# SIMPLE-BuildingSimulation/heat

Hardware: AMD Instinct MI355X
Metric: surface-node-updates/sec (higher is better)
Workload: dtype f64

## Files before the change

heat_amd/csrc/batch.hip:

```cpp
#include <hip/hip_runtime.h>
#include <rccl/rccl.h>

#include <dlfcn.h>

#include <algorithm>
#include <cmath>
#include <cstdarg>
#include <cstdio>
#include <cstdlib>
#include <cstring>
#include <limits>
#include <mutex>
#include <numeric>
#include <string>
#include <vector>

#include "../../include/heat_amd.h"
#include "kernels.hpp"
#include "layout.hpp"
#include "hostpool.hpp"
#include "plan.hpp"

using namespace heat;

// ... 492 lines not shown
    }

    SideArrays &sa = b->sa;
    sa.sc = b->d_side_const.p;
    sa.dyn = b->d_side_dyn.p;
    sa.out = b->d_side_out.p;
    sa.hs_fix = has_fix ? b->d_hs_fix.p : nullptr;
    sa.zc = b->d_zone_contrib.p;
    sa.S = (int32_t)S;
    sa.wstride = 0;
    sa.site = b->n_sites > 1 ? b->d_site.p : nullptr;
    NodeArrays &na = b->na;
    na.T = b->d_T.p; na.V = b->d_V.p; na.U = b->d_U.p;
    na.cls = b->d_cls.p; na.pal = b->d_pal.p;
    na.pal_stride = p.pal_stride;
    na.pal_ubase = p.pal_ubase;
    na.cavref = b->d_cavref.p; na.cavs = b->d_cavs.p;
    na.alpha_f = b->d_alpha_f.p; na.alpha_b = b->d_alpha_b.p; na.cav = b->d_cav_idx.p; na.mass = b->d_mass.p;
    SlotArrays &sl = b->sl;
    const int64_t *sp = b->d_slots.p;
    sl.hs_f = sp; sl.hs_b = sp + S; sl.flow_f = sp + 2 * S; sl.flow_b = sp + 3 * S;
    sl.solar_f = sp + 4 * S; sl.solar_b = sp + 5 * S; sl.ir_f = sp + 6 * S; sl.ir_b = sp + 7 * S;
    HIP_TRY(hipDeviceSynchronize());
    return HEAT_OK;
}

int select_device(heat_batch *b) {
    HIP_TRY(hipSetDevice(b->device));
    return HEAT_OK;
}

std::vector<FastTile> balanced_rounds(const std::vector<FastTile> &tiles, const std::vector<float> &cost, int n_waves) {
    const size_t n = tiles.size();
    if (n_waves <= 0 || n <= (size_t)n_waves) return tiles;
    std::vector<int32_t> order(n);
    std::iota(order.begin(), order.end(), 0);
    std::stable_sort(order.begin(), order.end(), [&](int32_t a, int32_t b) { return cost[a] > cost[b]; });
    std::vector<std::pair<float, int32_t>> heap(n_waves);
    for (int w = 0; w < n_waves; w++) heap[w] = {0.f, w};
    auto later = [](const std::pair<float, int32_t> &a, const std::pair<float, int32_t> &b) {
        return a.first > b.first || (a.first == b.first && a.second > b.second);
    };
    std::make_heap(heap.begin(), heap.end(), later);
    std::vector<std::vector<int32_t>> mine(n_waves);
    for (int32_t t : order) {
        std::pop_heap(heap.begin(), heap.end(), later);
        auto &top = heap.back();
        mine[top.second].push_back(t);
        top.first += cost[t];
        std::push_heap(heap.begin(), heap.end(), later);
    }
    size_t rounds = 0;
    for (const auto &m : mine) rounds = std::max(rounds, m.size());
    FastTile empty;
    empty.node_base = 0;
    empty.surf_base = 0;
    empty.k = (int16_t)(kStreamKindSmall << kStreamKindShift);
    empty.G = 0;
    std::vector<FastTile> out(rounds * (size_t)n_waves, empty);
    for (int w = 0; w < n_waves; w++)
        for (size_t r = 0; r < mine[w].size(); r++) out[r * (size_t)n_waves + w] = tiles[mine[w][r]];
    return out;
}

int rebuild_unified(heat_batch *b) {
    static const bool off = getenv("HEAT_AMD_NO_UNIFIED") != nullptr;
    auto eligible = [](int c) { return kFastPAL[c] && !(kFastM[c] == 16 && (kFastNM[c] || kFastCAV[c])); };
    static const bool cav_off = getenv("HEAT_AMD_NO_UNIFIED_CAV") != nullptr;
    size_t cap = (size_t)b->n_small_tiles;
    for (int c = 0; c < kNumFast; c++) if (eligible(c)) cap += b->h_tiles_cur[c].size();
    const int waves_light = b->n_cu * 3 * 4, waves_cav = b->n_cu * 2 * 4;
    cap += 2 * (size_t)(waves_light + waves_cav) + 2 * (size_t)(waves_light + waves_cav);
    if (b->d_ucount.n == 0) {
        b->ucount_stride = std::max<size_t>(cap, 1);
        HIP_TRY(b->d_ucount.zeros(2 * b->ucount_stride));
    }
    const int ns = b->n_small_plain_tiles;
    for (int c = 0; c < kNumFast; c++) {
        b->class_has_chunks[c] = false;
        for (const FastTile &ft : b->h_tiles_cur[c]) b->class_has_chunks[c] = b->class_has_chunks[c] || (ft.k & kTileChunkyBit) != 0;
    }
    for (int v = 0; v < 2; v++) {
        std::vector<FastTile> part[kStreamVariants];
        int n_classes = 0, n_cav_classes = 0;
        const int nsc = cav_off ? 0 : (v ? b->n_small_tiles - b->n_small_plain_tiles : b->n_smallcav_stream_tiles);
        for (int j = 0; j < nsc; j++) {
            const GeneralTile &g = b->h_gen_tiles_cur[b->n_small_plain_tiles + j];
            FastTile ft;
            ft.node_base = g.node_base;
            ft.surf_base = g.surf_base;
            ft.k = (int16_t)(kStreamKindSmall << kStreamKindShift);
            ft.G = (int16_t)g.G;
            part[3].push_back(ft);
        }
        for (int mi = 2; mi >= 0; mi--)
            for (int c = mi * 6; c < mi * 6 + 6; c++) {
                if (!eligible(c) || (kFastCAV[c] && cav_off)) continue;
                if (kFastCAV[c]) {
                    const int n = v ? b->n_fast_tiles[c] : b->n_stream_tiles[c];
                    n_cav_classes += n > 0;
                    for (int t = 0; t < n; t++) {
                        FastTile ft = b->h_tiles_cur[c][t];
                        ft.k = (int16_t)((ft.k & (0x1ff | kTileMixedBit | kTileChunkyBit)) | (mi << kStreamKindShift) | (kFastNM[c] ? kStreamNmBit : 0));
                        part[3].push_back(ft);
                    }
                    continue;
                }
                const int n = v ? b->n_fast_tiles[c] : b->n_stream_tiles[c];
                n_classes += n > 0;
                for (int t = 0; t < n; t++) {
                    FastTile ft = b->h_tiles_cur[c][t];
                    const bool chunks = (ft.k & kTileChunkyBit) != 0;
                    ft.k = (int16_t)((ft.k & (0x1ff | kTileMixedBit | kTileChunkyBit)) | (mi << kStreamKindShift) | (kFastNM[c] ? kStreamNmBit : 0));
                    part[mi == 2 ? 0 : (chunks ? 2 : 1)].push_back(ft);
                }
            }
        const bool use = !off && (n_classes + (ns > 0)) >= 2;
        const bool use_cav = !off && !cav_off && (n_cav_classes + (nsc > 0)) >= 2;
        b->n_ulist[v] = 0;
        for (int c = 0; c < kNumFast; c++) b->in_ulist[v][c] = eligible(c) && (kFastCAV[c] ? use_cav : use);
        b->small_in_ulist[v] = use && ns > 0;
        b->smallcav_in_ulist[v] = use_cav && nsc > 0;
        for (int q = 0; q < kStreamVariants; q++) b->ulist_part[v][q][0] = b->ulist_part[v][q][1] = 0;
        if (!use) part[0].clear(), part[1].clear(), part[2].clear();
        if (!use_cav) part[3].clear();
        if (!use && !use_cav) continue;
        static const bool balance_off = getenv("HEAT_AMD_NO_BALANCE") != nullptr;
        auto tile_cost = [&](const FastTile &ft, bool cav) -> float {
            const int kind = (ft.k >> kStreamKindShift) & 3;
            if (kind == kStreamKindSmall) return cav ? 12.f : 3.f;
            const float base = kind == 1 ? 1.f : 0.7f;
            if (cav) return 2.5f * base;
            return (ft.k & kStreamNmBit) ? 2.f * base : base;
        };
        if (use) {
            for (int j = 0; j < ns; j++) {
                const GeneralTile &g = b->h_gen_tiles_cur[j];
                FastTile ft;
                ft.node_base = g.node_base;
                ft.surf_base = g.surf_base;
                ft.k = (int16_t)(kStreamKindSmall << kStreamKindShift);
                ft.G = (int16_t)g.G;
                part[1].push_back(ft);
            }
        }
        for (int q : {1, 3}) {
            if (balance_off || part[q].empty()) continue;
            std::vector<float> cost(part[q].size());
            for (size_t t = 0; t < part[q].size(); t++) cost[t] = tile_cost(part[q][t], q == 3);
            part[q] = balanced_rounds(part[q], cost, q == 1 ? waves_light : waves_cav);
        }
        std::vector<FastTile> all;
        for (int q = 0; q < kStreamVariants; q++) {
            b->ulist_part[v][q][0] = (int)all.size();
            b->ulist_part[v][q][1] = (int)part[q].size();
            all.insert(all.end(), part[q].begin(), part[q].end());
        }
        if (all.size() > b->ucount_stride) return fail(HEAT_E_SIZE, "unified tile list grew beyond its counters");
        b->n_ulist[v] = (int)all.size();
        HIP_TRY(b->d_ulist[v].upload(all));
    }
    return HEAT_OK;
}

void enqueue_surfaces(heat_batch *b, int step_fixed, bool streamed_only = false) {
    int nt[kNumFast];
    for (int c = 0; c < kNumFast; c++) nt[c] = streamed_only ? b->n_stream_tiles[c] : b->n_fast_tiles[c];
    const int ul = streamed_only ? 0 : 1;
    const bool unified = b->n_ulist[ul] > 0;
    static const bool zigzag_off = getenv("HEAT_AMD_NO_ZIGZAG") != nullptr;
    const int rev = (!zigzag_off && (b->sweep_parity++ & 1)) ? 1 : 0;
    int n_small_plain = b->n_small_plain_tiles;
    if (unified) {
        for (int c = 0; c < kNumFast; c++) if (b->in_ulist[ul][c]) nt[c] = 0;
        if (b->small_in_ulist[ul]) n_small_plain = 0;
    }
    int n_launch = 0;
    for (int c = 0; c < kNumFast; c++) n_launch += nt[c] > 0;
    int n_cav_tiles = streamed_only ? b->n_smallcav_stream_tiles : b->n_small_tiles - b->n_small_plain_tiles;
    if (unified && b->smallcav_in_ulist[ul]) n_cav_tiles = 0;
    n_launch += unified;
    n_launch += n_small_plain > 0;
    n_launch += n_cav_tiles > 0;
    n_launch += b->n_gen_tiles > b->n_small_tiles;
    static const bool no_fork = getenv("HEAT_AMD_NO_FORK") != nullptr;
    const bool fork = n_launch > 1 && b->side[0] != nullptr && !no_fork && !b->capturing;
    const int n_side = fork ? std::min(n_launch - 1, (int)heat_batch::kSideStreams) : 0;
    int slot = 0;
    auto next_stream = [&]() -> hipStream_t {
        if (n_side == 0) return b->stream;
        const int s = slot++ % (n_side + 1);
        return s == 0 ? b->stream : b->side[s - 1];
    };
    if (n_side > 0) {
        (void)hipEventRecord(b->ev_fork, b->stream);
        for (int i = 0; i < n_side; i++) (void)hipStreamWaitEvent(b->side[i], b->ev_fork, 0);
    }
    if (unified) {
        hipStream_t us = next_stream();
        static const int order_env = getenv("HEAT_AMD_STREAM_ORDER") ? atoi(getenv("HEAT_AMD_STREAM_ORDER")) : 0;
        const int seq[2][kStreamVariants] = {{3, 1, 2, 0}, {0, 1, 2, 3}};
        for (int qi = 0; qi < kStreamVariants; qi++) {
            const int q = seq[order_env ? 1 : 0][rev ? kStreamVariants - 1 - qi : qi];
            const int first = b->ulist_part[ul][q][0], n = b->ulist_part[ul][q][1];
            if (n > 0)
                launch_surfaces_stream(q, b->d_ulist[ul].p + first, n, b->na, b->gen_base, b->sa, b->d_weather.p, b->d_step.p,
                                       step_fixed, b->d_zone_T.p, b->d_flags.p,
                                       b->d_ucount.p + ul * b->ucount_stride + first, b->n_cu, us, rev);
        }
    }
    double work[kNumFast], total_work = 0.0;
    for (int c = 0; c < kNumFast; c++) {
        work[c] = (double)nt[c] * kFastM[c];
        total_work += work[c];
    }
    total_work += 2.0 * b->n_gen_tiles;
    int order[kNumFast];
    for (int c = 0; c < kNumFast; c++) order[c] = c;
    std::sort(order, order + kNumFast, [&](int x, int y) { return nt[x] > nt[y]; });
    for (int q = 0; q < kNumFast; q++) {
        const int c = order[q];
        if (nt[c] <= 0) continue;
        launch_surfaces_fast(kFastM[c], kFastNM[c] ? (b->class_has_chunks[c] ? 2 : 1) : 0, kFastPAL[c], kFastCAV[c], work[c] / total_work,
                             b->d_fast_tiles[c].p, nt[c], b->na,
                             b->sa, b->d_weather.p, b->d_step.p, step_fixed, b->d_zone_T.p, b->d_flags.p,
                             b->d_nomass_iters.p + b->nm_count_base[c], b->n_cu, next_stream(), rev);
    }
    unsigned long long *cnt = b->d_nomass_iters.p + b->nm_count_base[kNumFast];
    if (n_small_plain > 0)
        launch_surfaces_small(0, b->d_gen_tiles.p, n_small_plain, b->na, b->gen_base, b->sa, b->d_cavs.p,
                              b->d_weather.p, b->d_step.p, step_fixed, b->d_zone_T.p, b->d_flags.p, cnt,
                              next_stream());
    if (n_cav_tiles > 0)
        launch_surfaces_small(1, b->d_gen_tiles.p + b->n_small_plain_tiles, n_cav_tiles,
                              b->na, b->gen_base, b->sa, b->d_cavs.p, b->d_weather.p, b->d_step.p, step_fixed,
                              b->d_zone_T.p, b->d_flags.p, cnt + (size_t)b->n_small_plain_tiles * kWave,
                              next_stream());
    if (b->n_gen_tiles > b->n_small_tiles)
        launch_surfaces_general(b->d_gen_tiles.p + b->n_small_tiles, b->n_gen_tiles - b->n_small_tiles, b->na,
                                b->gen_base, b->sa, b->d_cavs.p, b->d_scratch.p, b->d_weather.p, b->d_step.p,
                                step_fixed, b->d_zone_T.p, b->d_flags.p, cnt + (size_t)b->n_small_tiles * kWave,
                                next_stream());
    for (int i = 0; i < n_side; i++) {
        (void)hipEventRecord(b->ev_join[i], b->side[i]);
        (void)hipStreamWaitEvent(b->stream, b->ev_join[i], 0);
    }
}

void enqueue_zones(heat_batch *b, int mode) {
    const int32_t *zl = b->d_zlist.p;
    int nl = b->n_touched;
    if (mode == 3) { zl = b->d_stream_zones.p; nl = b->n_stream_zones; }
    if (mode == 5) { mode = 3; }
    if (mode == 4) { zl = b->d_zlist_stream.p; nl = b->n_touched_stream; mode = 2; }
    launch_zones(b->d_zone_off.p, b->d_zone_entries.p, b->d_zone_contrib.p, b->d_zone_a0.p, b->d_zone_b0.p,
                 b->d_zone_vol.p, b->d_zone_T.p, b->partial_ptr, (int)b->n_zones, b->dt, b->d_step.p,
                 b->d_flags.p, mode, zl, nl, b->d_slot_of.p, b->n_shared, b->zone_rows, b->stream);
}

int enqueue_fused(heat_batch *b, int n_sub, hipStream_t st, bool streamed_beside = false) {
    FusedArgs fa{};
    {
        static const bool zigzag_off = getenv("HEAT_AMD_NO_ZIGZAG") != nullptr;
        fa.reverse = (!zigzag_off && (b->fused_parity++ & 1)) ? 1 : 0;
    }
    fa.zones = b->d_fzones.p;
    fa.zone_eoff = b->d_fzone_eoff.p;
    fa.slots = b->d_fslots.p;
    fa.side_area = b->d_side_area.p;
    fa.side_lzone = b->d_side_lzone.p;
    fa.a0 = b->d_zone_a0.p;
    fa.b0 = b->d_zone_b0.p;
    fa.vol = b->d_zone_vol.p;
    fa.zone_T = b->d_zone_T.p;
    fa.dt = b->dt;
    fa.n_sub = n_sub;
    fa.gen_tiles = b->d_gen_tiles.p;
    fa.gen_base = b->gen_base;
    fa.small_iters = b->d_nomass_iters.p + b->nm_count_base[kNumFast];
    static const int reserve_env = getenv("HEAT_AMD_FUSED_RESERVE") ? atoi(getenv("HEAT_AMD_FUSED_RESERVE")) : -1;
    const bool beside_exchange = (b->comm != nullptr && b->shared_set && b->n_shared > 0) || reserve_env >= 0 || streamed_beside;
    double streamed_share = 0.0;
    if (streamed_beside) {
        double ns = 4.0 * kWave * (b->n_gen_tiles - (b->n_small_tiles - b->n_small_plain_tiles - b->n_smallcav_stream_tiles)), nf = 0.0;
        for (int c = 0; c < kNumFast; c++) {
            ns += (double)b->n_stream_tiles[c] * kFastM[c] * kWave;
            nf += (double)(b->n_fast_tiles[c] - b->n_stream_tiles[c]) * kFastM[c] * kWave;
        }
        streamed_share = ns / std::max(ns + nf, 1.0);
    }
    const int n_cu = b->n_cu;
    if (beside_exchange && b->d_fqueue.n == 0) HIP_TRY(b->d_fqueue.zeros(kNumFast * 4));
    for (int c = 0; c < kNumFast; c++)
        for (int g2 = 0; g2 < 4; g2++) {
            const int nb = (int)b->h_fblocks[c][g2].size();
            if (nb == 0) continue;
            fa.blocks = b->d_fblocks[c][g2].p;
            fa.n_blocks = nb;
            fa.queue = nullptr;
            int grid = nb;
            if (beside_exchange) {
                const int fw = (g2 & 1) ? 8 : 4;
                static const int room_env = getenv("HEAT_AMD_FUSED_ROOM") ? atoi(getenv("HEAT_AMD_FUSED_ROOM")) : 0;
                const int room = room_env > 0 ? room_env : n_cu * fused_blocks_per_cu(kFastM[c], kFastCAV[c], g2 >> 1, fw, b->na.pal_stride);
                const int reserve = reserve_env >= 0 ? reserve_env
                                                     : std::min(room / 2, std::max(fw == 4 ? 16 : 8, (int)(room * streamed_share)));
                if (nb > room - reserve) {
                    grid = std::max(1, room - reserve);
                    fa.queue = b->d_fqueue.p + c * 4 + g2;
                    HIP_TRY(hipMemsetAsync(fa.queue, 0, sizeof(unsigned int), st));
                }
            }
            static const bool trace = getenv("HEAT_AMD_TRACE") != nullptr;
            if (trace)
                fprintf(stderr, "heat_amd: fused launch%s: %d workgroups for %d blocks (class %d, list %d, %d sub-timesteps)\n",
                        fa.queue ? " on the work queue" : "", grid, nb, c, g2, n_sub);
            b->n_fused_launches++;
            const int nm_variant = kFastNM[c] ? ((b->class_has_chunks[c] && !(g2 >> 1) && !kFastCAV[c] && kFastM[c] <= 8) ? 2 : 1) : 0;
            HIP_TRY(launch_surfaces_fused(kFastM[c], nm_variant, kFastCAV[c], g2 >> 1, (g2 & 1) ? 8 : 4, grid, b->d_fast_tiles[c].p, b->n_fast_tiles[c],
                                          b->na, b->sa, b->d_weather.p, b->d_flags.p,
                                          b->d_nomass_iters.p + b->nm_count_base[c], fa, st));
        }
    for (int c = 0; c < kNumFast; c++) {
        const int n_super = (int)b->h_team_supers[c].size();
        if (n_super == 0) continue;
        if (n_sub > 4095) return fail(HEAT_E_INVALID_ARG, "a march call of %d sub-timesteps: the team exchange tags 4095 at most", n_sub);
        static const int team_room_env = getenv("HEAT_AMD_TEAM_ROOM") ? atoi(getenv("HEAT_AMD_TEAM_ROOM")) : 0;
        const int room = team_room_env > 0 ? team_room_env : n_cu * std::min(2, fused_team_blocks_per_cu(kFastM[c], kFastNM[c], b->na.pal_stride));
        int team_size = 2;
        for (const FusedSuper &su : b->h_team_supers[c]) team_size = std::max(team_size, (int)su.n_members);
        const int n_teams = std::min(n_super, std::max(0, room - room / 8) / team_size);
        if (n_teams >= 1 && (n_super + n_teams - 1) / n_teams > 1023)
            return fail(HEAT_E_SIZE, "%d clusters for %d teams: the exchange tags 1023 rounds per launch at most", n_super, n_teams);
        if (n_teams < 1) return fail(HEAT_E_DEVICE, "the device holds %d workgroups of the team variant: not one team", room);
        if (b->xbuf_teams < n_teams) {
            HIP_TRY(b->d_xbuf.zeros((size_t)n_teams * 2 * kTeamZones * kTeamMax * 4));
            b->xbuf_teams = n_teams;
        }
        b->team_epoch++;
        if ((b->team_epoch & 1023u) == 0) {
            HIP_TRY(hipMemsetAsync(b->d_xbuf.p, 0, b->d_xbuf.n * sizeof(unsigned long long), st));
            b->team_epoch++;
        }
        fa.blocks = b->d_team_blocks[c].p;
        fa.n_blocks = (int)b->h_team_blocks[c].size();
        fa.queue = nullptr;
        fa.supers = b->d_team_supers[c].p;
        fa.n_super = n_super;
        fa.team_zinfo = b->d_team_zinfo.p;
        fa.xbuf = b->d_xbuf.p;
        fa.tag_base = (b->team_epoch & 1023u) << 22;
        fa.team_size = team_size;
        static const bool trace = getenv("HEAT_AMD_TRACE") != nullptr;
        if (trace)
            fprintf(stderr, "heat_amd: team launch: %d teams of %d workgroups for %d clusters (class %d, %d sub-timesteps)\n",
                    n_teams, team_size, n_super, c, n_sub);
        b->n_fused_launches++;
        HIP_TRY(launch_surfaces_fused(kFastM[c], kFastNM[c], 0, 2, 4, n_teams * team_size, b->d_fast_tiles[c].p, b->n_fast_tiles[c], b->na,
                                      b->sa, b->d_weather.p, b->d_flags.p, b->d_nomass_iters.p + b->nm_count_base[c], fa, st));
    }
    return HEAT_OK;
}

hipEvent_t next_event(heat_batch *b) {
    if (b->ev_used == b->ev_pool.size()) {
        hipEvent_t e;
        if (hipEventCreate(&e) != hipSuccess) return nullptr;
        b->ev_pool.push_back(e);
    }
    return b->ev_pool[b->ev_used++];
}

struct MarchGuard {
    heat_batch *b;
    double *saved_partial;
    bool forked = false, joined = false;
    explicit MarchGuard(heat_batch *b_) : b(b_), saved_partial(b_->partial_ptr) {}
    ~MarchGuard() {
        b->partial_ptr = saved_partial;
        if (forked && !joined && b->fused_stream) (void)hipStreamSynchronize(b->fused_stream);
    }
};

struct SeriesDrain {
    heat_batch *b;
    ~SeriesDrain() { (void)hipStreamSynchronize(b->stream); }
};

template <typename T>
int series_upload(DevBuf<T> &buf, const T *src, size_t count, const char *what) {
    hipError_t e = buf.alloc(count);
    if (e == hipSuccess && count > 0) e = hipMemcpy(buf.p, src, count * sizeof(T), hipMemcpyHostToDevice);
    if (e != hipSuccess)
        return fail(HEAT_E_DEVICE, "series march: %s (%zu bytes) on the device: %s — nothing has been marched", what, count * sizeof(T),
                    hipGetErrorString(e));
    return HEAT_OK;
}

struct ReportDev {
    DevBuf<uint8_t> gbuf, prev;
    DevBuf<uint32_t> gidx, seg, part_off;
    DevBuf<double> gw, part, group_trace, applied_row;
    DevBuf<double> f64[7];
    DevBuf<int64_t> i64[4];
    DevBuf<double> th_f64[2];
    DevBuf<int64_t> th_i64[3];
};

struct IdealDev {
    DevBuf<int32_t> i32;
    DevBuf<double> cap;
    DevBuf<double> step;
    DevBuf<double> q;
    DevBuf<double> f64[4];
    DevBuf<int64_t> i64[4];
};

struct SkyDev {
    DevBuf<uint8_t> mode;
    DevBuf<double> normal;
    DevBuf<SkyRecord> record;
};
static_assert(sizeof(SkyRecord) == sizeof(heat_sky_record) && sizeof(heat_sky_record) == 64, "SkyRecord mirrors heat_sky_record");

struct GainsDev {
    DevBuf<int32_t> ap_dev;
    DevBuf<double> ap_f64;
    DevBuf<double2> power;
    DevBuf<double> sum;
    DevBuf<double> transmitted;
    DevBuf<uint32_t> rec;
    DevBuf<int64_t> slice_off;
    DevBuf<int32_t> ap;
    DevBuf<double> share;
};

struct AirDev {
    DevBuf<int32_t> i32;
    DevBuf<double> f64;
    DevBuf<uint8_t> state;
    DevBuf<double> sum_q;
    DevBuf<int64_t> i64[2];
    DevBuf<double> path_q;
};

struct ShadeDev {
    DevBuf<double> tab;
    DevBuf<int32_t> i32;
    DevBuf<double> tan2;
    DevBuf<double> f;
    DevBuf<int32_t> side;
    DevBuf<int32_t> aperture;
    DevBuf<double> sunlit;
};

struct RadiationDev {
    DevBuf<uint32_t> face;
    DevBuf<double> emission;
    DevBuf<uint32_t> rec;
    DevBuf<int32_t> off, src;
    DevBuf<double> factor;
    DevBuf<double> sum;
    DevBuf<double> irradiance;
};

template <typename T>
int series_alloc(DevBuf<T> &buf, size_t count, const char *what) {
    const hipError_t e = buf.alloc(count);
    if (e != hipSuccess)
        return fail(HEAT_E_DEVICE, "series march: %s (%zu bytes) on the device: %s — nothing has been marched", what, count * sizeof(T),
                    hipGetErrorString(e));
    return HEAT_OK;
}
template <typename T>
int report_array(DevBuf<T> &buf, const T *host, size_t count, bool upload, const char *what) {
    if (!host) return HEAT_OK;
    return upload ? series_upload(buf, host, count, what) : series_alloc(buf, count, what);
}

}

extern "C" {


int heat_batch_create(const heat_batch_desc *desc, heat_batch **out) {
    heat_batch_options opt;
    memset(&opt, 0, sizeof opt);
    opt.device = -1;
    opt.n_ranks = 1;
    return heat_batch_create_ex(desc, &opt, out);
}

static int create_impl(const heat_batch_desc *desc, const heat_batch_options *opt_in, int32_t n_sites,
                       const int32_t *site_of_surface, bool sites, heat_batch **out) {
    if (!out) return fail(HEAT_E_INVALID_ARG, "out is NULL");
    *out = nullptr;
    heat_batch_options opt;
    memset(&opt, 0, sizeof opt);
    opt.device = -1;
    opt.n_ranks = 1;
    if (opt_in) opt = *opt_in;
    if (sites) {
        std::string err;
        const int rc = check_sites(desc, opt, n_sites, site_of_surface, err);
        if (rc) return fail(rc, "%s", err.c_str());
    }
    if (opt.n_ranks < 1) opt.n_ranks = 1;
    if (opt.nodes_per_lane != 0 && opt.nodes_per_lane != 4 && opt.nodes_per_lane != 8 && opt.nodes_per_lane != 16)
        return fail(HEAT_E_INVALID_ARG, "nodes_per_lane must be 0, 4, 8 or 16");
    int rc;
    {
        std::string err;
        rc = check_desc(desc, err);
        if (rc) return fail(rc, "%s", err.c_str());
    }

    int ndev = 0;
    if (hipGetDeviceCount(&ndev) != hipSuccess || ndev == 0)
        return fail(HEAT_E_DEVICE, "no HIP device available: this library has no CPU fallback");
    heat_batch *b = new heat_batch();
    if (opt.device >= 0) {
        b->device = opt.device;
    } else if (hipGetDevice(&b->device) != hipSuccess) {
        delete b;
        return fail(HEAT_E_DEVICE, "hipGetDevice failed");
    }
    b->n_ranks = opt.n_ranks;
    b->rank = opt.rank;
    b->use_graph = opt.use_graph != 0;
    b->fusion_on = opt.no_fusion != 1;
    rc = select_device(b);
    if (!rc) {
        hipDeviceProp_t prop;
        if (hipGetDeviceProperties(&prop, b->device) == hipSuccess && prop.multiProcessorCount > 0) b->n_cu = prop.multiProcessorCount;
    }
    if (!rc) {
        if (opt.stream) {
            b->stream = reinterpret_cast<hipStream_t>(opt.stream);
        } else {
            hipError_t e = hipStreamCreateWithFlags(&b->stream, hipStreamNonBlocking);
            if (e != hipSuccess) rc = fail(HEAT_E_DEVICE, "hipStreamCreate failed: %s", hipGetErrorString(e));
            b->own_stream = true;
        }
    }
    if (!rc) {
        for (int i = 0; i < heat_batch::kSideStreams && !rc; i++) {
            if (hipStreamCreateWithFlags(&b->side[i], hipStreamNonBlocking) != hipSuccess ||
                hipEventCreateWithFlags(&b->ev_join[i], hipEventDisableTiming) != hipSuccess)
                rc = fail(HEAT_E_DEVICE, "side stream creation failed");
        }
        if (!rc && hipStreamCreateWithFlags(&b->fused_stream, hipStreamNonBlocking) != hipSuccess)
            rc = fail(HEAT_E_DEVICE, "side stream creation failed");
        if (!rc && (hipEventCreateWithFlags(&b->ev_fork, hipEventDisableTiming) != hipSuccess ||
                    hipEventCreateWithFlags(&b->ev_fused, hipEventDisableTiming) != hipSuccess))
            rc = fail(HEAT_E_DEVICE, "event creation failed");
    }
    if (!rc) rc = build(b, desc, opt, n_sites, site_of_surface);
    if (rc) {
        delete b;
        return rc;
    }
    *out = b;
    return HEAT_OK;
}

int heat_batch_create_ex(const heat_batch_desc *desc, const heat_batch_options *opt, heat_batch **out) {
    return create_impl(desc, opt, 1, nullptr, false, out);
}

int heat_batch_create_sites(const heat_batch_desc *desc, const heat_batch_options *opt, int32_t n_sites,
                            const int32_t *site_of_surface, heat_batch **out) {
    return create_impl(desc, opt, n_sites, site_of_surface, true, out);
}

int32_t heat_batch_n_sites(const heat_batch *b) { return b ? b->n_sites : 0; }

int heat_batch_create_shard(const heat_batch_desc *desc, const heat_batch_options *opt, const int32_t *rank_of_surface,
                            heat_batch **out) {
    if (!desc || !opt || !rank_of_surface || !out) return fail(HEAT_E_INVALID_ARG, "NULL argument");
    {
        std::string err;
        const int rc = check_desc(desc, err);
        if (rc) return fail(rc, "%s", err.c_str());
    }
    for (int64_t s = 0; s < desc->n_surfaces; s++)
        if (rank_of_surface[s] < 0 || rank_of_surface[s] >= std::max(opt->n_ranks, 1))
            return fail(HEAT_E_SIZE, "surface %lld: rank %d outside [0, %d)", (long long)s, rank_of_surface[s], std::max(opt->n_ranks, 1));
    ShardDesc sh;
    sh.build(desc, rank_of_surface, opt->rank);
    int rc = heat_batch_create_ex(&sh.desc, opt, out);
    if (rc) return rc;
    heat_batch *b = *out;
    const int64_t Z = desc->n_zones;
    const int n_ranks = std::max(opt->n_ranks, 1);
    std::vector<int32_t> first(Z, -1);
    std::vector<uint8_t> shared(Z, 0), owned(Z, 0);
    auto touch = [&](int32_t z, int32_t rk) {
        if (first[z] < 0) first[z] = rk;
        else if (first[z] != rk) shared[z] = 1;
    };
    for (int64_t s = 0; s < desc->n_surfaces; s++) {
        if (desc->front_kind[s] == HEAT_BOUNDARY_SPACE) touch(desc->front_zone[s], rank_of_surface[s]);
        if (desc->back_kind[s] == HEAT_BOUNDARY_SPACE) touch(desc->back_zone[s], rank_of_surface[s]);
    }
    int64_t n_shared = 0;
    for (int64_t z = 0; z < Z; z++) {
        n_shared += shared[z];
// ... 1508 lines not shown
```

heat_amd/csrc/device_math.hpp:

```cpp
#pragma once
#include <hip/hip_runtime.h>
#include "layout.hpp"

namespace heat {

constexpr double kPi = 3.14159265358979323846264338327950288;

__device__ __forceinline__ double tarp_natural(double air_t, double surf_t, double cos_tilt, int &bad) {
    const double delta_t = air_t - surf_t;
    const double adt = fabs(delta_t);
    const double act = fabs(cos_tilt);
    const double c3 = cbrt(adt);
    double h;
    if (adt < 1e-3 || act < 1e-3) {
        h = 1.31 * c3;
    } else if ((delta_t < 0. && cos_tilt < 0.) || (delta_t > 0. && cos_tilt > 0.)) {
        h = 9.482 * c3 / (7.238 - act);
    } else if ((delta_t > 0. && cos_tilt < 0.) || (delta_t < 0. && cos_tilt > 0.)) {
        h = 1.81 * c3 / (1.382 + act);
    } else {
        bad |= FLAG_UNREACHABLE;
        h = __builtin_nan("");
    }
    return (h < 0.1) ? 0.1 : h;
}

__device__ __forceinline__ double tarp_natural_coef(double air_t, double surf_t, double nat_pos, double nat_neg, int &bad) {
    const double delta_t = air_t - surf_t;
    const double adt = fabs(delta_t);
    const double c3 = cbrt(adt);
    double coef = (delta_t > 0.) ? nat_pos : nat_neg;
    if (adt < 1e-3) coef = 1.31;
    if (delta_t != delta_t || nat_pos != nat_pos) {
        bad |= FLAG_UNREACHABLE;
        coef = __builtin_nan("");
    }
    const double h = coef * c3;
    return (h < 0.1) ? 0.1 : h;
}

__device__ __forceinline__ double tarp_forced(double air_speed, double area, double perimeter, bool windward) {
    const double wf = windward ? 1.0 : 0.5;
    return 2.537 * wf * 1.67 * sqrt(perimeter * air_speed / area);
}

__device__ __forceinline__ bool is_windward(double sin_wd, double cos_wd, double cos_tilt, double nx, double ny) {
    return (fabs(cos_tilt) < 0.98) ? ((nx * sin_wd + ny * cos_wd) > 0.0) : true;
}

__device__ __forceinline__ double ir_to_rad_temperature(double ir) {
    return sqrt(sqrt(ir / kSigma)) - 273.15;
}

__device__ __forceinline__ double clamp_solar_front(double s) { return (s != s || s < 0.0) ? 0.0 : s; }
__device__ __forceinline__ double clamp_solar_back(double s) { return (s != s) ? 0.0 : s; }

__device__ __forceinline__ double rad_hs(double emis, double rad_t, double surf_t) {
    const double tm = 273.15 + (rad_t + surf_t) / 2.;
    return 4. * emis * kSigma * ((tm * tm) * tm);
}

__device__ __forceinline__ void gas_coeffs(int gas, double &k0, double &k1, double &m0, double &m1,
                                           double &c0, double &c1, double &mass) {
    switch (gas) {
    case 1: k0 = 2.285e-3; k1 = 5.149e-5; m0 = 3.379e-6; m1 = 6.451e-8; c0 = 521.9285; c1 = 0.; mass = 39.948; break;
    case 2: k0 = 9.443e-4; k1 = 2.826e-5; m0 = 2.213e-6; m1 = 7.777e-8; c0 = 248.0907; c1 = 0.; mass = 83.8; break;
    case 3: k0 = 4.538e-4; k1 = 1.723e-5; m0 = 1.069e-6; m1 = 7.414e-8; c0 = 158.3397; c1 = 0.; mass = 131.30; break;
    default: k0 = 2.873e-3; k1 = 7.760e-5; m0 = 3.723e-6; m1 = 4.94e-8; c0 = 1002.7370; c1 = 1.2324e-2; mass = 28.97; break;
    }
}

__device__ __forceinline__ double air_density(double temp_k) {
    return 101325. * 28.97 / (8314.46261815324 * temp_k);
}
__device__ __forceinline__ double air_heat_capacity(double temp_k) {
    return 1002.7370 + 1.2324e-2 * temp_k;
}
__device__ __forceinline__ double zone_mcp(double volume, double temp) {
    return volume * air_density(temp + 273.15) * air_heat_capacity(temp + 273.15) / 1.;
}

__device__ __forceinline__ double powr(double x, double y) { return exp(y * log(x)); }

__device__ __attribute__((noinline)) double nu_90(double ra, double a_gi, int &bad) {
    double nu1;
    if (ra <= 1e4) {
        nu1 = 1. + 1.7596678 * 1e-10 * powr(ra, 2.2984755);
    } else if (ra < 5e4) {
        nu1 = 0.028154 * powr(ra, 0.4134);
    } else if (ra > 5e4) {
        nu1 = 0.0673838 * cbrt(ra);
    } else {
        bad |= FLAG_UNREACHABLE;
        nu1 = __builtin_nan("");
    }
    const double nu2 = 0.242 * powr(ra / a_gi, 0.272);
    return (nu1 > nu2) ? nu1 : nu2;
}

__device__ __attribute__((noinline)) double nu_60(double ra, double a_gi) {
    const double g = 0.5 / powr(1. + powr(ra / 3160., 20.6), 0.1);
    const double t = 0.0936 * powr(ra, 0.314) / (1. + g);
    const double t2 = t * t, t4 = t2 * t2;
    const double t7 = (t * t2) * t4;
    const double nu1 = powr(1. + t7, 1. / 7.);
    const double nu2 = (0.104 + 0.175 / a_gi) * powr(ra, 0.283);
    return (nu1 > nu2) ? nu1 : nu2;
}

__device__ __attribute__((noinline)) double nusselt(double ra, double gamma, double a_gi, int &bad) {
    const double THIRTY_RAD = 30. * kPi / 180.;
    const double EPSILON_RAD = 0.5 * kPi / 180.;
    gamma = fmod(gamma, kPi);
    if (gamma >= 0.0 && gamma < 2. * THIRTY_RAD - EPSILON_RAD) {
        const double cos_gamma = cos(gamma);
        const double x = 1. - 1708. / (ra * cos_gamma);
        const double a = (x + fabs(x)) / 2.;
        const double b = 1. - 1708. * powr(sin(1.8 * gamma), 1.6) / (ra * cos_gamma);
        const double c = cbrt(ra * cos_gamma / 5830.) - 1.;
        return 1. + 1.44 * a * b + (c + fabs(c)) / 2.;
    } else if (gamma < 2. * THIRTY_RAD + EPSILON_RAD) {
        return nu_60(ra, a_gi);
    } else if (gamma < 3. * THIRTY_RAD - EPSILON_RAD) {
        const double nu60 = nu_60(ra, a_gi);
        const double nu90 = nu_90(ra, a_gi, bad);
        const double x = (gamma - kPi / 3.) / (kPi / 2. - kPi / 3.);
        return nu60 + (nu90 - nu60) * x;
    } else if (gamma < 3. * THIRTY_RAD + EPSILON_RAD) {
        return nu_90(ra, a_gi, bad);
    } else if (gamma < 6. * THIRTY_RAD) {
        const double nu_v = nu_90(ra, a_gi, bad);
        return 1. + (nu_v - 1.) * sin(gamma);
    }
    bad |= FLAG_UNREACHABLE;
    return __builtin_nan("");
}

__device__ inline double cavity_u_value(const CavityDev &c, double t_front, double t_back, int &bad) {
    double k0, k1, m0, m1, c0, c1, mass;
    gas_coeffs(c.gas, k0, k1, m0, m1, c0, c1, mass);
    double gamma = c.angle;
    if (t_front > t_back) gamma = 180. * (kPi / 180.) - gamma;
    const double a_gi = c.height / c.thickness;
    const double temp = ((t_front + 273.15) + (t_back + 273.15)) / 2.;
    const double lambda = k0 + k1 * temp;
    double ra;
    if (fabs(t_front - t_back) < 1e-10) {
        ra = 0.0000001;
    } else {
        const double beta = 1. / temp;
        const double c_p = (c1 != 0.) ? c0 + c1 * temp : c0;
        const double mu = m0 + m1 * temp;
        const double rho = 101325. * mass / (8314.46261815324 * temp);
        const double th = c.thickness;
        ra = (rho * rho) * ((th * th) * th) * 9.81 * beta * c_p * fabs(t_front - t_back) / (mu * lambda);
    }
    const double nu = nusselt(ra, gamma, a_gi, bad);
    const double conv = nu * lambda / c.thickness;
    const double tm = (t_back + t_front) / 2. + 273.15;
    const double rad = 4. * ((tm * tm) * tm) * kSigma * c.ein * c.eout / (1. - (1. - c.ein) * (1. - c.eout));
    return rad + conv;
}

}
```

heat_amd/csrc/kernels.hip:

```cpp
#include <hip/hip_runtime.h>

#include <algorithm>
#include <atomic>
#include <cstdlib>

#include "device_math.hpp"
#include "kernels.hpp"
#include "layout.hpp"

namespace heat {

__device__ __forceinline__ void eval_side(const SideConst &c, const StepWeather &w, double air_t, double rad_alt,
                                          double rad_out, double surf_t, double &hs, double &rad_t, int &bad) {
    const double natural = tarp_natural(air_t, surf_t, c.cos_eff, bad);
    if ((c.kind_n & 3) == KIND_OUTDOOR) {
        const bool windward = (c.kind_n & 4) ? true : ((c.nx * w.sin_wd + c.ny * w.cos_wd) > 0.0);
        const double wf = windward ? 1.0 : 0.5;
        hs = wf * (c.forced * w.sqrt_ws) + natural;
        rad_t = rad_out;
    } else {
        hs = natural;
        rad_t = rad_alt;
    }
}

typedef __attribute__((address_space(4))) const int32_t ConstInt32;
__device__ __forceinline__ int tile_site(const SideArrays &sd, int surf_base) {
    const ConstInt32 *site = (const ConstInt32 *)sd.site;
    return __builtin_amdgcn_readfirstlane(site[__builtin_amdgcn_readfirstlane(surf_base)]);
}
__device__ __forceinline__ const StepWeather *site_weather(const StepWeather *weather, const SideArrays &sd, int surf_base) {
    if (sd.site == nullptr) return weather;
    return weather + (int64_t)tile_site(sd, surf_base) * sd.wstride;
}

__device__ __forceinline__ double boundary_temperature(const SideConst &c, const StepWeather &w,
                                                       const double *__restrict__ zone_T) {
    const int kind = c.kind_n & 3;
    if (kind == KIND_SPACE) return zone_T[c.zone];
    if (kind == KIND_AMBIENT) return c.ambient;
    return w.t_out;
}

__device__ __forceinline__ long long side_entry_pos(const SideConst &c) { return __double_as_longlong(c.ambient); }
__device__ __forceinline__ void put_zone_contrib(const SideArrays &sd, const SideConst &c, double hs, double t_face) {
    if ((c.kind_n & 3) == KIND_SPACE) {
        ZoneContrib z;
        z.ha = hs * c.forced;
        z.t_face = t_face;
        sd.zc[side_entry_pos(c)] = z;
    }
}

__device__ __forceinline__ void report_failure(int *flags, int bad, unsigned int index) {
    atomicOr(flags, bad);
    atomicMin(reinterpret_cast<unsigned long long *>(flags + 2), ((unsigned long long)index << 8) | (unsigned int)(bad & 0xff));
}

__device__ __forceinline__ double shfl_f64(double v, int src_lane) { return __shfl(v, src_lane, kWave); }

template <int CTRL>
__device__ __forceinline__ double dpp_rotate_f64(double v) {
    int lo = __double2loint(v), hi = __double2hiint(v);
    lo = __builtin_amdgcn_update_dpp(0, lo, CTRL, 0xf, 0xf, false);
    hi = __builtin_amdgcn_update_dpp(0, hi, CTRL, 0xf, 0xf, false);
    return __hiloint2double(hi, lo);
}
template <int CTRL, int ROW_MASK>
__device__ __forceinline__ double dpp_add_f64(double v) {
    int lo = __double2loint(v), hi = __double2hiint(v);
    lo = __builtin_amdgcn_update_dpp(0, lo, CTRL, ROW_MASK, 0xf, true);
    hi = __builtin_amdgcn_update_dpp(0, hi, CTRL, ROW_MASK, 0xf, true);
    return v + __hiloint2double(hi, lo);
}
__device__ __forceinline__ double wave_sum_f64(double v) {
    v = dpp_add_f64<0x111, 0xf>(v);
    v = dpp_add_f64<0x112, 0xf>(v);
    v = dpp_add_f64<0x114, 0xf>(v);
    v = dpp_add_f64<0x118, 0xf>(v);
    v = dpp_add_f64<0x142, 0xa>(v);
    v = dpp_add_f64<0x143, 0xc>(v);
    const int lo = __builtin_amdgcn_readlane(__double2loint(v), 63);
    const int hi = __builtin_amdgcn_readlane(__double2hiint(v), 63);
    return __hiloint2double(hi, lo);
}

__device__ __forceinline__ double row_sum_f64(double v) {
    v = dpp_add_f64<0x111, 0xf>(v);
    v = dpp_add_f64<0x112, 0xf>(v);
    v = dpp_add_f64<0x114, 0xf>(v);
    v = dpp_add_f64<0x118, 0xf>(v);
    return v;
}

__device__ __forceinline__ double from_prev_lane(double v) { return dpp_rotate_f64<0x13C>(v); }
__device__ __forceinline__ double from_next_lane(double v) { return dpp_rotate_f64<0x134>(v); }

template <int M, bool AFFINE, typename VF, typename QF, typename PUT>
__device__ __forceinline__ void apply_A(const double (&x)[M], VF V, const double (&Ue)[M], double ULe, bool is_first,
                                        bool is_last, double qF, QF qsel, PUT put) {
    const double xl_raw = from_prev_lane(x[M - 1]);
    const double xr_raw = from_next_lane(x[0]);
    const double xl = is_first ? 0.0 : xl_raw;
    const double xr = is_last ? 0.0 : xr_raw;
    double fprev = ULe * (x[0] - xl);
    if (AFFINE) fprev -= qF;
#pragma unroll
    for (int j = 0; j < M; j++) {
        const double xj = x[j];
        double f = Ue[j] * (((j == M - 1) ? xr : x[j + 1]) - xj);
        if (AFFINE) f += qsel(j);
        put(j, V(j) * (f - fprev));
        fprev = f;
    }
}

template <int M, typename VF, typename QF>
__device__ __forceinline__ void rk4_horner(double (&T)[M], VF V, const double (&Ue)[M], double ULe, bool is_first,
                                           bool is_last, double qF, QF qsel) {
    double v[M], z[M];
    apply_A<M, true>(T, V, Ue, ULe, is_first, is_last, qF, qsel, [&](int j, double y) { v[j] = y * (1.0 / 24.0); });
    apply_A<M, false>(v, V, Ue, ULe, is_first, is_last, qF, qsel, [&](int j, double y) { z[j] = 4.0 * v[j] + y; });
    apply_A<M, false>(z, V, Ue, ULe, is_first, is_last, qF, qsel, [&](int j, double y) { z[j] = 12.0 * v[j] + y; });
    apply_A<M, false>(z, V, Ue, ULe, is_first, is_last, qF, qsel,
                      [&](int j, double y) { T[j] = (T[j] + 24.0 * v[j]) + y; });
}

#pragma clang fp contract(off)
constexpr int kSmallNodes = 4;
__device__ __forceinline__ double opaque_select(bool cond, double x, double y) {
    const unsigned long long m = __builtin_amdgcn_ballot_w64(cond);
    int lo, hi;
    asm("v_cndmask_b32 %0, %1, %2, %3" : "=v"(lo) : "v"(__double2loint(y)), "v"(__double2loint(x)), "s"(m));
    asm("v_cndmask_b32 %0, %1, %2, %3" : "=v"(hi) : "v"(__double2hiint(y)), "v"(__double2hiint(x)), "s"(m));
    return __hiloint2double(hi, lo);
}
struct Nodes4 {
    double a, b, c, d;
    __device__ __forceinline__ double get(int j) const { return j == 0 ? +a : (j == 1 ? +b : (j == 2 ? +c : +d)); }
    __device__ __forceinline__ void set(int j, double v) {
        if (j == 0) a = v;
        else if (j == 1) b = v;
        else if (j == 2) c = v;
        else d = v;
    }
    __device__ __forceinline__ double last(int nn) const {
        double r = a;
        r = opaque_select(nn == 2, b, r);
        r = opaque_select(nn == 3, c, r);
        r = opaque_select(nn == 4, d, r);
        return r;
    }
};

template <int CAV>
__device__ __forceinline__ void small_step(const SideConst &cf, const SideConst &cb, const SideDyn &df, const SideDyn &db,
                                           const double *__restrict__ hs_fix, int d, int S, const StepWeather &w,
                                           double t_front_b, double t_back_b, int nn, Nodes4 &T,
                                           const double (&Us)[kSmallNodes], const double (&sol)[kSmallNodes],
                                           const int (&cav)[kSmallNodes], const CavityDev (&cv)[kSmallNodes - 1], int &bad,
                                           unsigned int &iters, SideOut &of, SideOut &ob) {
    constexpr int NS = kSmallNodes;
    const int bk = cb.kind_n & 3;
    auto last = [&](const double (&x)[NS]) {
        double r = x[0];
#pragma unroll
        for (int j = 1; j < NS; j++) r = (j == nn - 1) ? +x[j] : +r;
        return r;
    };
    const double T0 = T.a, Tn = T.last(nn);
    const bool quirk = (bk == KIND_AMBIENT);
    double f_hs, f_rad, b_hs, b_rad;
    const double f_surf = T0, b_surf = quirk ? T0 : Tn;
    eval_side(cf, w, t_front_b, t_front_b, df.rad_t, f_surf, f_hs, f_rad, bad);
    eval_side(cb, w, t_back_b, quirk ? t_front_b : t_back_b, db.rad_t, b_surf, b_hs, b_rad, bad);
    if (f_hs != f_hs || b_hs != b_hs) bad |= FLAG_NAN_HS;
    if (hs_fix != nullptr) {
        const double ff = hs_fix[d], fb = hs_fix[S + d];
        if (ff == ff) f_hs = ff;
        if (fb == fb) b_hs = fb;
    }
    const double f_radhs = rad_hs(cf.emis, f_rad, f_surf);
    const double b_radhs = rad_hs(cb.emis, b_rad, b_surf);

    double old_err = 99999.;
    int count = 0;
    for (;;) {
        double lo[NS], dg[NS], up[NS], q[NS];
#pragma unroll
        for (int j = 0; j < NS; j++) { lo[j] = 0.0; dg[j] = 0.0; up[j] = 0.0; q[j] = 0.0; }
#pragma unroll
        for (int j = 0; j < NS - 1; j++) {
            if (j < nn - 1) {
                double u = Us[j];
                if constexpr (CAV) {
                    if (cav[j] >= 0) u = cavity_u_value(cv[j], T.get(j), T.get(j + 1), bad);
                }
                dg[j] += -u;
                dg[j + 1] = dg[j + 1] - u;
                up[j] = up[j] + u;
                lo[j + 1] = lo[j + 1] + u;
            }
        }
        q[0] += t_front_b * f_hs + f_radhs * (f_rad - T.a);
        dg[0] += -f_hs;
        const double bq = t_back_b * b_hs + b_radhs * (b_rad - T.last(nn));
#pragma unroll
        for (int j = 0; j < NS; j++) {
            if (j == nn - 1) { q[j] += bq; dg[j] += -b_hs; }
        }
        iters++;
#pragma unroll
        for (int j = 0; j < NS; j++) q[j] = (q[j] + sol[j]) * -1.;
#pragma unroll
        for (int j = 1; j < NS; j++) {
            if (j < nn) {
                const double f = lo[j] / dg[j - 1];
                dg[j] -= f * up[j - 1];
                q[j] -= f * q[j - 1];
            }
        }
        double x[NS];
#pragma unroll
        for (int j = NS - 1; j >= 0; j--) {
            if (j == nn - 1) x[j] = q[j] / dg[j];
            else if (j < nn - 1) x[j] = (q[j] - up[j] * x[(j + 1) % NS]) / dg[j];
            else x[j] = 0.0;
        }
        double err = 0.0;
#pragma unroll
        for (int j = 0; j < NS; j++) if (j < nn) err += fabs(x[j] - T.get(j));
        if (err > old_err) break;
        if (err != err) { bad |= FLAG_NAN_NOMASS; break; }
#pragma unroll
        for (int j = 0; j < NS; j++) if (j < nn) T.set(j, (T.get(j) + x[j]) * 0.5);
        const double tol = (count < 100) ? 0.01 : 0.5;
        if (err / (double)nn < tol) break;
        old_err = err;
        count++;
    }

    {
        const double T0n = T.a, Tnn = T.last(nn);
        double fh, bh, r_;
        eval_side(cf, w, t_front_b, t_front_b, df.rad_t, T0n, fh, r_, bad);
        eval_side(cb, w, t_back_b, t_back_b, db.rad_t, quirk ? T0n : Tnn, bh, r_, bad);
        if (fh != fh || bh != bh) bad |= FLAG_NAN_HS;
        if (hs_fix != nullptr) {
            const double ff = hs_fix[d], fb = hs_fix[S + d];
            if (ff == ff) fh = ff;
            if (fb == fb) bh = fb;
        }
        of.hs = fh; of.flow = (T0n - t_front_b) * fh;
        ob.hs = bh; ob.flow = (Tnn - t_back_b) * bh;
    }
}

template <int CAV>
__device__ __forceinline__ void small_load(const GeneralTile &tile, int lane, const NodeArrays &na, int64_t gen_base,
                                           const SideDyn &df, const SideDyn &db, int nn, Nodes4 &T,
                                           double (&Us)[kSmallNodes], double (&sol)[kSmallNodes], int (&cav)[kSmallNodes],
                                           CavityDev (&cv)[kSmallNodes - 1]) {
    const double *Tg = na.T + tile.node_base + lane;
    const double *Ug = na.U + tile.node_base + lane;
    const int64_t gofs = tile.node_base - gen_base + lane;
    double tl[kSmallNodes], ul[kSmallNodes], af[kSmallNodes], ab[kSmallNodes];
    int cl[kSmallNodes];
#pragma unroll
    for (int j = 0; j < kSmallNodes; j++) {
        const int64_t jc = (int64_t)min(j, nn - 1) * kWave;
        tl[j] = Tg[jc];
        ul[j] = Ug[jc];
        af[j] = na.alpha_f[gofs + jc];
        ab[j] = na.alpha_b[gofs + jc];
        cl[j] = CAV ? na.cav[gofs + jc] : -1;
    }
#pragma unroll
    for (int j = 0; j < kSmallNodes; j++) {
        const bool v = j < nn;
        T.set(j, v ? tl[j] : 0.0);
        Us[j] = v ? ul[j] : 0.0;
        cav[j] = (CAV && v) ? cl[j] : -1;
        double sj = v ? af[j] * df.solar : 0.0;
        sj += v ? ab[j] * db.solar : 0.0;
        sol[j] = sj;
    }
#pragma unroll
    for (int j = 0; j < kSmallNodes - 1; j++) {
        cv[j] = CavityDev{0., 0., 0., 0., 0., 0, 0};
        if constexpr (CAV) {
            if (cav[j] >= 0) cv[j] = na.cavs[cav[j]];
        }
    }
}

template <int CAV>
__device__ __forceinline__ unsigned int small_tile_march(int64_t node_base, int surf_base, int G, int lane,
                                                         const NodeArrays &na, int64_t gen_base, const SideArrays &sd,
                                                         const StepWeather &w, const double *__restrict__ zone_T,
                                                         int *__restrict__ flags) {
    if (lane >= G) return 0;
    GeneralTile tile;
    tile.node_base = node_base;
    tile.surf_base = surf_base;
    tile.G = G;
    const int d = surf_base + lane;
    const int S = sd.S;
    const SideConst cf = sd.sc[d];
    const SideConst cb = sd.sc[S + d];
    const SideDyn df = sd.dyn[d];
    const SideDyn db = sd.dyn[S + d];
    const int nn = cf.kind_n >> 16;
    Nodes4 T{0.0, 0.0, 0.0, 0.0};
    double Us[kSmallNodes], sol[kSmallNodes];
    int cav[kSmallNodes];
    CavityDev cv[kSmallNodes - 1];
    small_load<CAV>(tile, lane, na, gen_base, df, db, nn, T, Us, sol, cav, cv);
    int bad = 0;
    unsigned int iters = 0;
    SideOut of, ob;
    small_step<CAV>(cf, cb, df, db, sd.hs_fix, d, S, w, boundary_temperature(cf, w, zone_T),
                    boundary_temperature(cb, w, zone_T), nn, T, Us, sol, cav, cv, bad, iters, of, ob);
    double *Tg = na.T + node_base + lane;
#pragma unroll
    for (int j = 0; j < kSmallNodes; j++) if (j < nn) Tg[(int64_t)j * kWave] = T.get(j);
    sd.out[d] = of;
    sd.out[S + d] = ob;
    {
        const double Tl = T.last(nn);
        put_zone_contrib(sd, cf, of.hs, T.a);
        put_zone_contrib(sd, cb, ob.hs, Tl);
    }
    if (bad) report_failure(flags, bad, (unsigned int)d);
    return iters;
}

template <int CAV>
__global__ void __launch_bounds__(256, 2)
k_surfaces_small(const GeneralTile *__restrict__ tiles, int n_tiles, NodeArrays na, int64_t gen_base,
                 SideArrays sd, const CavityDev *__restrict__ cavs,
                 const StepWeather *__restrict__ weather, const int *__restrict__ step_ptr, int step_fixed,
                 const double *__restrict__ zone_T, int *__restrict__ flags,
                 unsigned long long *__restrict__ nomass_iters) {
    const int lane = threadIdx.x & (kWave - 1);
    const int wave = blockIdx.x * (blockDim.x >> 6) + (threadIdx.x >> 6);
    if (wave >= n_tiles) return;
    const GeneralTile tile = tiles[wave];
    const int step = (step_fixed >= 0) ? step_fixed : *step_ptr;
    const StepWeather w = site_weather(weather, sd, tile.surf_base)[step];
    const unsigned int iters = small_tile_march<CAV>(tile.node_base, tile.surf_base, tile.G, lane, na, gen_base, sd, w, zone_T, flags);
    if (lane < tile.G) nomass_iters[(int64_t)wave * kWave + lane] += iters;
}
#pragma clang fp contract(fast)

struct FusedLds {
    double2 *hT;
    double *zT, *za0, *zb0, *zvol;
    double *zsa, *zsb;
    int *zoff;
    unsigned short *slots;
};

constexpr int kFusedBarriersAtInit = 1;
constexpr int kFusedBarriersPerSubstep = 2;

__device__ __forceinline__ void fused_block_init(const FusedBlock &blk, const FusedArgs &fa, const FusedLds &l, int n_threads) {
    const int e_first = fa.zone_eoff[blk.first_zone];
    if ((int)threadIdx.x <= blk.n_zones) l.zoff[threadIdx.x] = fa.zone_eoff[blk.first_zone + threadIdx.x] - e_first;
    if ((int)threadIdx.x < blk.n_zones) {
        const int z = fa.zones[blk.first_zone + threadIdx.x];
        l.zT[threadIdx.x] = fa.zone_T[z];
        l.za0[threadIdx.x] = fa.a0[z];
        l.zb0[threadIdx.x] = fa.b0[z];
        l.zvol[threadIdx.x] = fa.vol[z];
    }
    const int n_e = fa.zone_eoff[blk.first_zone + blk.n_zones] - e_first;
    for (int e = threadIdx.x; e < n_e; e += n_threads) l.slots[fa.slots[e_first + e]] = (unsigned short)e;
    __syncthreads();
}

struct FusedPre {
    int e_first, n_e, zoff, z, slot0;
    double zT, za0, zb0, zvol;
};
__device__ __forceinline__ void fused_pre_a(const FusedBlock &blk, const FusedArgs &fa, FusedPre &p) {
    p = FusedPre{0, 0, 0, 0, 0, 0.0, 0.0, 0.0, 0.0};
    const int nz = blk.n_zones;
    if (nz > 0) {
        p.e_first = fa.zone_eoff[blk.first_zone];
        p.n_e = fa.zone_eoff[blk.first_zone + nz];
        p.zoff = fa.zone_eoff[blk.first_zone + min((int)threadIdx.x, nz)];
        p.z = fa.zones[blk.first_zone + min((int)threadIdx.x, nz - 1)];
    }
}
__device__ __forceinline__ void fused_pre_b(const FusedBlock &blk, const FusedArgs &fa, FusedPre &p) {
    if (blk.n_zones > 0) {
        p.n_e -= p.e_first;
        p.zoff -= p.e_first;
        p.zT = fa.zone_T[p.z];
        p.za0 = fa.a0[p.z];
        p.zb0 = fa.b0[p.z];
        p.zvol = fa.vol[p.z];
        if (p.n_e > 0) p.slot0 = fa.slots[p.e_first + min((int)threadIdx.x, p.n_e - 1)];
    }
}
__device__ __forceinline__ void fused_block_init(const FusedBlock &blk, const FusedArgs &fa, const FusedLds &l, int n_threads,
                                                 const FusedPre &p) {
    if ((int)threadIdx.x <= blk.n_zones) l.zoff[threadIdx.x] = p.zoff;
    if ((int)threadIdx.x < blk.n_zones) {
        l.zT[threadIdx.x] = p.zT;
        l.za0[threadIdx.x] = p.za0;
        l.zb0[threadIdx.x] = p.zb0;
        l.zvol[threadIdx.x] = p.zvol;
    }
    if ((int)threadIdx.x < p.n_e) l.slots[p.slot0] = (unsigned short)threadIdx.x;
    for (int e = threadIdx.x + n_threads; e < p.n_e; e += n_threads) l.slots[fa.slots[p.e_first + e]] = (unsigned short)e;
    __syncthreads();
}

struct TeamCtx {
    int team, member, round, it;
    int *flags;
};
__device__ __forceinline__ unsigned long long team_granule(unsigned int data, unsigned int tag) {
    return ((unsigned long long)tag << 32) | data;
}
template <int TEAM>
__device__ __forceinline__ void fused_zone_phase(const FusedBlock &blk, const FusedArgs &fa, const FusedLds &l, int wib,
                                                 int n_waves, int lane, int &bad_all, const TeamCtx &tc_) {
    __syncthreads();
    auto team_area = [&](int j, unsigned int &mask, unsigned int &tag) -> unsigned long long * {
        const unsigned int info = fa.team_zinfo[blk.first_zone + j];
        mask = info >> 16;
        tag = fa.tag_base | ((unsigned int)tc_.round << 12) | (unsigned int)(tc_.it + 1);
        return fa.xbuf + ((((size_t)tc_.team * 2 + (tc_.it & 1)) * kTeamZones + (info & 0xffffu)) * kTeamMax) * 4;
    };
    auto publish = [&](int j, double a, double b) {
        unsigned int mask, tag;
        unsigned long long *g = team_area(j, mask, tag) + tc_.member * 4;
        const unsigned long long ab = (unsigned long long)__double_as_longlong(a), bb = (unsigned long long)__double_as_longlong(b);
        __hip_atomic_store(g + 0, team_granule((unsigned int)ab, tag), __ATOMIC_RELAXED, __HIP_MEMORY_SCOPE_AGENT);
        __hip_atomic_store(g + 1, team_granule((unsigned int)(ab >> 32), tag), __ATOMIC_RELAXED, __HIP_MEMORY_SCOPE_AGENT);
        __hip_atomic_store(g + 2, team_granule((unsigned int)bb, tag), __ATOMIC_RELAXED, __HIP_MEMORY_SCOPE_AGENT);
        __hip_atomic_store(g + 3, team_granule((unsigned int)(bb >> 32), tag), __ATOMIC_RELAXED, __HIP_MEMORY_SCOPE_AGENT);
    };
    auto gather = [&](int j, double &a, double &b) {
        unsigned int mask, tag;
        const unsigned long long *area = team_area(j, mask, tag);
        double sa = 0.0, sb = 0.0;
        for (int m = 0; m < kTeamMax; m++) {
            if (!((mask >> m) & 1u)) continue;
            double am = a, bm = b;
            if (m != tc_.member) {
                const unsigned long long *g = area + m * 4;
                unsigned long long g0 = 0, g1 = 0, g2 = 0, g3 = 0;
                bool got = false;
                for (int spin = 0; spin < (1 << 21); spin++) {
                    g0 = __hip_atomic_load(g + 0, __ATOMIC_RELAXED, __HIP_MEMORY_SCOPE_AGENT);
                    g1 = __hip_atomic_load(g + 1, __ATOMIC_RELAXED, __HIP_MEMORY_SCOPE_AGENT);
                    g2 = __hip_atomic_load(g + 2, __ATOMIC_RELAXED, __HIP_MEMORY_SCOPE_AGENT);
                    g3 = __hip_atomic_load(g + 3, __ATOMIC_RELAXED, __HIP_MEMORY_SCOPE_AGENT);
                    got = (unsigned int)(g0 >> 32) == tag && (unsigned int)(g1 >> 32) == tag &&
                          (unsigned int)(g2 >> 32) == tag && (unsigned int)(g3 >> 32) == tag;
                    if (got) break;
                    __builtin_amdgcn_s_sleep(4);
                }
                if (!got) atomicOr(tc_.flags, FLAG_EXCHANGE);
                am = __longlong_as_double((long long)((g0 & 0xffffffffull) | (g1 << 32)));
                bm = __longlong_as_double((long long)((g2 & 0xffffffffull) | (g3 << 32)));
            }
            sa += am;
            sb += bm;
        }
        a = sa;
        b = sb;
    };
    auto finish = [&](int j, double a, double b, double tc, double cz) {
        a += l.za0[j];
        b += l.zb0[j];
        double ft = tc;
        if (fabs(b) > 1e-9) ft = a / b + (tc - a / b) * exp(-b * fa.dt / cz);
        if (ft != ft) bad_all |= FLAG_NAN_ZONE;
        l.zT[j] = ft;
    };
    if (blk.n_zones <= n_waves) {
        if (wib < blk.n_zones) {
            const int j = wib;
            const int e0 = l.zoff[j], e1 = l.zoff[j + 1];
            const double tc = l.zT[j];
            const double cz = zone_mcp(l.zvol[j], tc);
            double a = 0.0, b = 0.0;
            for (int e = e0 + lane; e < e1; e += kWave) {
                const double2 ht = l.hT[e];
                a += ht.x * ht.y;
                b += ht.x;
            }
            a = wave_sum_f64(a);
            b = wave_sum_f64(b);
            if (lane == 0) {
                if constexpr (TEAM) {
                    publish(j, a, b);
                    gather(j, a, b);
                }
                finish(j, a, b, tc, cz);
            }
        }
    } else {
        const int row = lane >> 4, rl = lane & 15;
        const bool one_pass = blk.n_zones <= 4 * n_waves;
        (void)one_pass;
#pragma clang loop unroll(disable)
        for (int j0 = 0; j0 < blk.n_zones; j0 += 4 * n_waves) {
            const int j = j0 + 4 * wib + row;
            const bool on = j < blk.n_zones;
            const int jj = on ? j : 0;
            const int e0 = l.zoff[jj], e1 = on ? l.zoff[jj + 1] : e0;
            const double tc = l.zT[jj];
            const double cz = zone_mcp(l.zvol[jj], tc);
            double a = 0.0, b = 0.0;
            for (int e = e0 + rl; __any(e < e1); e += 16) {
                if (e < e1) {
                    const double2 ht = l.hT[e];
                    a += ht.x * ht.y;
                    b += ht.x;
                }
            }
            a = row_sum_f64(a);
            b = row_sum_f64(b);
            if constexpr (TEAM) {
                if (on && rl == 15) {
                    publish(j, a, b);
                    if (one_pass) {
                        gather(j, a, b);
                        finish(j, a, b, tc, cz);
                    } else {
                        l.zsa[j] = a;
                        l.zsb[j] = b;
                    }
                }
            } else {
                if (on && rl == 15) finish(j, a, b, tc, cz);
            }
        }
        if constexpr (TEAM) {
            if (!one_pass) {
#pragma clang loop unroll(disable)
                for (int j0 = 0; j0 < blk.n_zones; j0 += 4 * n_waves) {
                    const int j = j0 + 4 * wib + row;
                    if (j < blk.n_zones && rl == 15) {
                        const double tc = l.zT[j];
                        const double cz = zone_mcp(l.zvol[j], tc);
                        double a = l.zsa[j], b = l.zsb[j];
                        gather(j, a, b);
                        finish(j, a, b, tc, cz);
                    }
                }
            }
        }
    }
    __syncthreads();
}

#pragma clang fp contract(off)
__device__ void fused_small_wave(const FusedBlock &blk, const FusedArgs &fa, const FusedLds &l, int lanes_per_side,
                                 int wib, int n_waves, int lane, const NodeArrays &na, const SideArrays &sd,
                                 const StepWeather *__restrict__ weather, int *__restrict__ flags) {
    const int tile_index = blk.first_small + (wib - blk.n_tiles);
    const GeneralTile tile = fa.gen_tiles[tile_index];
    weather = site_weather(weather, sd, tile.surf_base);
    const bool active = lane < tile.G;
    const int d = tile.surf_base + (active ? lane : 0);
    const int S = sd.S;
    const SideConst cf = sd.sc[d];
    const SideConst cb = sd.sc[S + d];
    const SideDyn df = sd.dyn[d];
    const SideDyn db = sd.dyn[S + d];
    const int nn = cf.kind_n >> 16;
    const int lz_f = fa.side_lzone[d], lz_b = fa.side_lzone[S + d];
    const double area = fa.side_area[d];
    Nodes4 T{0.0, 0.0, 0.0, 0.0};
    double Us[kSmallNodes], sol[kSmallNodes];
    int cav[kSmallNodes];
    CavityDev cv[kSmallNodes - 1];
    small_load<1>(tile, active ? lane : 0, na, fa.gen_base, df, db, nn, T, Us, sol, cav, cv);
    fused_block_init(blk, fa, l, n_waves * kWave);
    int bad_all = 0;
    unsigned int iters = 0;
    SideOut of{0.0, 0.0}, ob{0.0, 0.0};
    auto btemp = [&](const SideConst &c, int lz, const StepWeather &w) -> double {
        const int kind = c.kind_n & 3;
        if (kind == KIND_SPACE) return l.zT[lz];
        if (kind == KIND_AMBIENT) return c.ambient;
        return w.t_out;
    };
#pragma clang loop unroll(disable)
    for (int it = 0; it < fa.n_sub; it++) {
        const StepWeather w = weather[it];
        int bad = 0;
        small_step<1>(cf, cb, df, db, sd.hs_fix, d, S, w, btemp(cf, lz_f, w), btemp(cb, lz_b, w), nn, T, Us, sol, cav,
                      cv, bad, iters, of, ob);
        if (active) {
            bad_all |= bad;
            const double Tl = T.last(nn);
            if ((cf.kind_n & 3) == KIND_SPACE) l.hT[l.slots[wib * kWave + lane]] = make_double2(of.hs * area, T.a);
            if ((cb.kind_n & 3) == KIND_SPACE) l.hT[l.slots[lanes_per_side + wib * kWave + lane]] = make_double2(ob.hs * area, Tl);
        }
        fused_zone_phase<0>(blk, fa, l, wib, n_waves, lane, bad_all, TeamCtx{0, 0, 0, 0, nullptr});
    }
    if ((int)threadIdx.x < blk.n_zones) fa.zone_T[fa.zones[blk.first_zone + threadIdx.x]] = l.zT[threadIdx.x];
    if (active) {
        double *Tg = na.T + tile.node_base + lane;
#pragma unroll
        for (int j = 0; j < kSmallNodes; j++) if (j < nn) Tg[(int64_t)j * kWave] = T.get(j);
        sd.out[d] = of;
        sd.out[S + d] = ob;
        if (fa.small_iters) fa.small_iters[(int64_t)tile_index * kWave + lane] += iters;
    }
    if (bad_all) report_failure(flags, bad_all, (unsigned int)d);
}
#pragma clang fp contract(fast)

#ifdef HEAT_STAMPS
constexpr int kStampsPerBlock = 8;
__device__ unsigned long long g_stamps[65536 * kStampsPerBlock];
#define HEAT_STAMP(k, real)                                                                                   \
    do {                                                                                                      \
        if constexpr (FUSED) {                                                                                \
            if (threadIdx.x == 0 && (counter_index >> 2) < 65536)                                             \
                g_stamps[(counter_index >> 2) * kStampsPerBlock + (k)] =                                      \
                    (real) ? __builtin_amdgcn_s_memrealtime() : __builtin_amdgcn_s_memtime();                 \
        }                                                                                                     \
    } while (0)
#else
#define HEAT_STAMP(k, real) do { } while (0)
#endif
#ifdef HEAT_STREAM_STAMPS
#ifndef HEAT_STAMPS
constexpr int kStampsPerBlock = 8;
__device__ unsigned long long g_stamps[65536 * kStampsPerBlock];
#endif
#define HEAT_SSTAMP(k, drain)                                                                                  \
    do {                                                                                                       \
        if constexpr (!FUSED && PAL) {                                                                         \
            if (drain) asm volatile("s_waitcnt vmcnt(0) lgkmcnt(0)" ::: "memory");                             \
            if (lane == 0 && counter_index < 32768)                                                            \
                g_stamps[(counter_index + (M == 16 ? 32768 : 0)) * kStampsPerBlock + (k)] = __builtin_amdgcn_s_memtime(); \
        }                                                                                                      \
    } while (0)
#else
#define HEAT_SSTAMP(k, drain) do { } while (0)
#endif

template <int M, int NM, int PAL, int CAV, int FUSED, int SMALL = 0>
__device__ __forceinline__ void fast_tile_march(const FastTile tile, int counter_index, bool nm_on, int lane, int wib,
                                                double *s_pal, double *s_V, double *s_pos, const FusedLds &fl, const FusedBlock &blk,
                                                int blk_waves, int n_it, int step0, const NodeArrays &na,
                                                const SideArrays &sd, const StepWeather *__restrict__ weather,
                                                const double *__restrict__ zone_T, int *__restrict__ flags,
                                                unsigned long long *__restrict__ nomass_iters, const FusedArgs &fa,
                                                bool write_out = true, const TeamCtx team = TeamCtx{0, 0, 0, 0, nullptr}) {
    constexpr int kLanes = (FUSED ? FUSED : 4) * kWave;
    constexpr bool kVinLds = FUSED && M == 16;
    HEAT_STAMP(4, true);
    HEAT_STAMP(0, false);
    HEAT_SSTAMP(0, false);
    double2 *const s_hT = fl.hT;
    double *const s_zT = fl.zT;
    (void)s_hT; (void)s_zT; (void)s_V; (void)s_pos; (void)nm_on; (void)blk; (void)blk_waves; (void)counter_index;
    FusedPre pre;
    (void)pre;
    if constexpr (FUSED) fused_pre_a(blk, fa, pre);
    const bool mixed = PAL && (tile.k & kTileMixedBit) != 0;
    constexpr bool kChunks = NM == 2 && PAL;
    const bool chunky = kChunks && (tile.k & kTileChunkyBit) != 0;
    const int k = tile.k & 0xff;
    const bool full = (tile.k & 0x100) != 0;
    const int G = tile.G;
    const int Lk = mixed ? k : (kWave / k) * k;
    int g = (int)(((float)lane + 0.5f) * (1.0f / (float)k));
    int seg = lane - g * k;
    bool is_last = (seg == k - 1);
    const bool in_layout = lane < Lk;
    if (mixed) {
        const unsigned int e = reinterpret_cast<const unsigned short *>(na.cls + tile.node_base + (int64_t)M * Lk)[in_layout ? lane : 0];
        g = (int)(e & 63u);
        seg = (int)((e >> 6) & 63u);
        is_last = (e & (unsigned int)kLaneLastBit) != 0;
    }
    const bool active = in_layout && (g < G);
    if (!active) g = 0;
    const int d = tile.surf_base + g;
    const int ll = in_layout ? lane : 0;

    const int S = sd.S;
    const bool is_first = (seg == 0);
    constexpr bool kSingleLane = !FUSED || (M == 8 && !CAV);
    const bool single = kSingleLane && is_first && is_last;
    const bool my_back = !is_first;
    const int sidx = (my_back ? S : 0) + d;
    const SideConst c_load = sd.sc[sidx];
    const SideDyn dy_load = sd.dyn[sidx];
    SideConst cb2 = c_load;
    SideDyn db2 = dy_load;
    if constexpr (kSingleLane) {
        if ((!mixed && k == 1) || single) {
            cb2 = sd.sc[S + d];
            db2 = sd.dyn[S + d];
        }
    }
    int4 cavref = make_int4(-1, -1, -1, -1);
    if constexpr (CAV) cavref = reinterpret_cast<const int4 *>(na.cavref)[d];
    const int kind_n_mine = c_load.kind_n;
    if constexpr (!FUSED) s_pos[threadIdx.x] = c_load.ambient;
    int my_lz = 0, b_lz = 0;
    double my_area = 0.0;
    if constexpr (FUSED) {
        my_lz = fa.side_lzone[sidx];
        my_area = fa.side_area[sidx];
        if constexpr (kSingleLane) b_lz = single ? fa.side_lzone[S + d] : 0;
    }
    (void)b_lz;
    int peer_lz = 0;
    if constexpr (FUSED) peer_lz = fa.side_lzone[d];
    (void)peer_lz;

    double T[M], V[M], U[M];
    unsigned int cw[M / 4];
    (void)cw;
    if constexpr (PAL) {
        const int pstride = na.pal_stride;
        const int ubase = na.pal_ubase;
        double *sp = s_pal + wib * (kWave * pstride);
        auto load_cls_T = [&]() {
            const unsigned char *pc = na.cls + tile.node_base + (int64_t)ll * M;
            if constexpr (M == 4) {
                cw[0] = *reinterpret_cast<const unsigned int *>(pc);
            } else {
#pragma unroll
                for (int q = 0; q < M / 8; q++) {
                    const uint2 w0 = reinterpret_cast<const uint2 *>(pc)[q];
                    cw[2 * q] = w0.x;
                    cw[2 * q + 1] = w0.y;
                }
            }
            const double2 *pT = reinterpret_cast<const double2 *>(na.T + tile.node_base);
#pragma unroll
            for (int jp = 0; jp < M / 2; jp++) {
                const double2 t = pT[jp * Lk + ll];
                T[2 * jp] = t.x; T[2 * jp + 1] = t.y;
            }
        };
        if constexpr (FUSED) {
            load_cls_T();
            fused_pre_b(blk, fa, pre);
        }
        {
            const double2 *gp = reinterpret_cast<const double2 *>(na.pal + (int64_t)tile.surf_base * pstride);
            double2 *sp2 = reinterpret_cast<double2 *>(sp);
            const int n2 = G * (pstride / 2);
            for (int i0 = 0; i0 < n2; i0 += 6 * kWave) {
                double2 t6[6];
#pragma unroll
                for (int q = 0; q < 6; q++) t6[q] = gp[min(i0 + q * kWave + lane, n2 - 1)];
                if constexpr (FUSED) {
                    asm volatile("" : "+v"(t6[0].x), "+v"(t6[1].x), "+v"(t6[2].x), "+v"(t6[3].x), "+v"(t6[4].x), "+v"(t6[5].x),
                                      "+v"(pre.zT), "+v"(pre.za0), "+v"(pre.zb0), "+v"(pre.zvol), "+v"(pre.slot0));
                }
#pragma unroll
                for (int q = 0; q < 6; q++)
                    if (i0 + q * kWave + lane < n2) sp2[i0 + q * kWave + lane] = t6[q];
            }
        }
        if constexpr (!FUSED) load_cls_T();
        HEAT_STAMP(6, false);
        __builtin_amdgcn_wave_barrier();
        {
            const double *mp = sp + g * pstride;
#pragma unroll
            for (int j = 0; j < M; j++) {
                const unsigned int cbj = (cw[j >> 2] >> (8 * (j & 3))) & 0xff;
                const unsigned int vi = cbj & (kPalV - 1);
                V[j] = mp[vi >= kPalVMark1 ? 0u : vi];
                U[j] = mp[ubase + ((cbj >> kPalUShift) & (kPalU - 1))];
            }
        }
        if constexpr (kVinLds) {
#pragma unroll
            for (int j = 0; j < M; j++) s_V[j * kLanes + threadIdx.x] = V[j];
        }
    } else {
        const double2 *pT = reinterpret_cast<const double2 *>(na.T + tile.node_base);
        const double2 *pV = reinterpret_cast<const double2 *>(na.V + tile.node_base);
        const double2 *pU = reinterpret_cast<const double2 *>(na.U + tile.node_base);
#pragma unroll
        for (int jp = 0; jp < M / 2; jp++) {
            const double2 t = pT[jp * Lk + ll];
            const double2 v = pV[jp * Lk + ll];
            const double2 u = pU[jp * Lk + ll];
            T[2 * jp] = t.x; T[2 * jp + 1] = t.y;
            V[2 * jp] = v.x; V[2 * jp + 1] = v.y;
            U[2 * jp] = u.x; U[2 * jp + 1] = u.y;
        }
    }
    HEAT_STAMP(7, false);
    if constexpr (FUSED) fused_block_init(blk, fa, fl, blk_waves * kWave, pre);

    const int first_lane = lane - seg;
    const int nn = kind_n_mine >> 16;
    const int jl = full ? (M - 1) : (nn - 1 - (mixed ? seg : k - 1) * M);

    auto pick_last = [&](const double (&x)[M]) {
        double r = x[M - 1];
        if (!full) {
#pragma unroll
            for (int j = 0; j < M - 1; j++) r = (j == jl) ? +x[j] : +r;
        }
        return r;
    };

    const bool wave_quirk = __any((is_last && (kind_n_mine & 3) == KIND_AMBIENT && my_back) ||
                                  (single && ((kind_n_mine >> 4) & 3) == KIND_AMBIENT));
    double zt_mine = 0.0, zt_b2 = 0.0;
    (void)zt_mine; (void)zt_b2;
    if constexpr (!FUSED) {
        zt_mine = zone_T[c_load.zone];
        if constexpr (kSingleLane) zt_b2 = zone_T[cb2.zone];
    }

    auto Vat = [&](int j) -> double {
        if constexpr (kVinLds) return s_V[j * kLanes + threadIdx.x];
        else return V[j];
    };
    auto V_last = [&]() {
        double r = Vat(M - 1);
        if (!full) {
#pragma unroll
            for (int j = 0; j < M - 1; j++) r = (j == jl) ? Vat(j) : r;
        }
        return r;
    };

    int bad_all = 0;
    unsigned int nm_passes = 0;
    double o_hs = 0.0, o_flow = 0.0, o2_hs = 0.0, o2_flow = 0.0;
    StepWeather w_next = weather[step0];

    HEAT_STAMP(1, false);
    HEAT_SSTAMP(1, true);
    SideConst c_cur = c_load;
    SideDyn dy_cur = dy_load;
#pragma clang loop unroll(disable)
    for (int it = 0; it < n_it; it++) {
    const StepWeather w = w_next;
    if constexpr (FUSED) w_next = weather[min(it + 1, n_it - 1)];
    const SideConst c = c_cur;
    const SideDyn dy = dy_cur;
    auto btemp = [&](const SideConst &cc, int lz, double zt) -> double {
        const int kind = cc.kind_n & 3;
        if (kind == KIND_SPACE) {
            if constexpr (FUSED) return s_zT[lz];
            else return zt;
        }
        if (kind == KIND_AMBIENT) return cc.ambient;
        return w.t_out;
    };

    int bad = 0;
    auto prepare = [&](const SideConst &cc, const SideDyn &dd, bool back, int rec, int lz, double zt, double &air_t,
                       double &rad_t, double &forced, bool &use_front_T) {
        const int kind = cc.kind_n & 3;
        air_t = btemp(cc, lz, zt);
        rad_t = air_t;
        use_front_T = false;
        forced = 0.0;
        if (kind == KIND_OUTDOOR) {
            const bool windward = (cc.kind_n & 4) ? true : ((cc.nx * w.sin_wd + cc.ny * w.cos_wd) > 0.0);
            forced = (windward ? 1.0 : 0.5) * (cc.forced * w.sqrt_ws);
            rad_t = dd.rad_t;
        } else if (back && kind == KIND_AMBIENT) {
            const int fkind = (cc.kind_n >> 4) & 3;
            if (fkind == KIND_SPACE) {
                if constexpr (FUSED) rad_t = s_zT[peer_lz];
                else rad_t = zt;
            } else if (fkind == KIND_AMBIENT) {
                rad_t = cc.forced;
            } else {
                rad_t = w.t_out;
            }
            use_front_T = true;
        }
        (void)rec;
    };
    auto conv = [&](double air_t, double forced, double nat_pos, double nat_neg, int rec, double surf_t) {
        double hs = forced + tarp_natural_coef(air_t, surf_t, nat_pos, nat_neg, bad);
        if (hs != hs) bad |= FLAG_NAN_HS;
        if (sd.hs_fix != nullptr) {
            const double fix = sd.hs_fix[rec];
            if (fix == fix) hs = fix;
        }
        return hs;
    };

    const double T0 = wave_quirk ? shfl_f64(T[0], first_lane) : T[0];
    const double Tn = pick_last(T);

    double UL = from_prev_lane(U[M - 1]);
    if (is_first) UL = 0.0;
    double T_prev_last = 0.0;
    if constexpr (NM) T_prev_last = from_prev_lane(T[M - 1]);

    double hF = 0.0, qF = 0.0, hB = 0.0, qB = 0.0;
    double fF_hs = 0.0, fF_rhs = 0.0, fF_rad = 0.0, fF_air = 0.0, fF_sol = 0.0;
    double fB_hs = 0.0, fB_rhs = 0.0, fB_rad = 0.0, fB_air = 0.0, fB_sol = 0.0;
    (void)fF_hs; (void)fF_rhs; (void)fF_rad; (void)fF_air; (void)fF_sol;
    (void)fB_hs; (void)fB_rhs; (void)fB_rad; (void)fB_air; (void)fB_sol;
    auto add_face = [&](const SideConst &cc, const SideDyn &dd, bool back, double air_t, double rad_t, double forced,
                        int rec, bool use_front_T, double &h_out, double &q_out) {
        h_out = 0.0;
        q_out = 0.0;
        const double surf_t = (back && !use_front_T) ? Tn : T0;
        const double hs = conv(air_t, forced, cc.cos_eff, cc.alpha, rec, surf_t);
        const double rhs = rad_hs(cc.emis, rad_t, surf_t);
        const double sol = dd.solar;
        if constexpr (NM) {
            if constexpr (kChunks) {
                fF_hs = back ? fF_hs : hs; fF_rhs = back ? fF_rhs : rhs; fF_rad = back ? fF_rad : rad_t;
                fF_air = back ? fF_air : air_t; fF_sol = back ? fF_sol : sol;
                fB_hs = back ? hs : fB_hs; fB_rhs = back ? rhs : fB_rhs; fB_rad = back ? rad_t : fB_rad;
                fB_air = back ? air_t : fB_air; fB_sol = back ? sol : fB_sol;
            }
            const double vface = back ? V_last() : Vat(0);
            if (nm_on && active && vface == 0.0 && nn >= 2) {
                if (chunky) return;
                double u_in, t_in;
                if (!back) {
                    u_in = U[0];
                    t_in = T[1 % M];
                } else {
                    double up = UL, tp = T_prev_last;
#pragma unroll
                    for (int j = 1; j < M; j++) {
                        up = (j == jl) ? +U[j - 1] : +up;
                        tp = (j == jl) ? +T[j - 1] : +tp;
                    }
                    u_in = up;
                    t_in = tp;
                }
                double Tc = back ? pick_last(T) : T[0];
                const double dg = (0.0 - hs) - u_in;
                const double nb = u_in * t_in;
                double old_err = 99999.;
                int count = 0;
                for (;;) {
                    const double qf = air_t * hs + rhs * (rad_t - Tc);
                    const double q = ((back ? (nb + qf) : (qf + nb)) + sol) * -1.;
                    const double x = q / dg;
                    const double err = fabs(x - Tc);
                    nm_passes++;
                    if (err > old_err) break;
                    if (err != err) { bad |= FLAG_NAN_NOMASS; break; }
                    Tc = (Tc + x) * 0.5;
                    const double tol = (count < 100) ? 0.01 : 0.5;
                    if (err < tol) break;
                    old_err = err;
                    count++;
                }
                if (!back) {
                    T[0] = Tc;
                } else {
#pragma unroll
                    for (int j = 0; j < M; j++) T[j] = (j == jl) ? Tc : T[j];
                }
                return;
            }
        }
        const double tface = back ? pick_last(T) : T[0];
        h_out = hs;
        q_out = (air_t * hs + rhs * (rad_t - tface)) + sol;
    };

    double my_air, my_rad, my_forced;
    bool my_useF;
    prepare(c, dy, my_back, sidx, my_lz, zt_mine, my_air, my_rad, my_forced, my_useF);
    if (is_first || is_last) {
        double h_, q_;
        add_face(c, dy, my_back, my_air, my_rad, my_forced, sidx, my_useF, h_, q_);
        hF = my_back ? 0.0 : h_;
        qF = my_back ? 0.0 : q_;
        hB = my_back ? h_ : 0.0;
        qB = my_back ? q_ : 0.0;
    }
    double b_air = 0.0, b_forced = 0.0, b_cos = 0.0, b_neg = 0.0;
    bool b_useF = false;
    if constexpr (kSingleLane) {
        if (single) {
            double b_rad;
            prepare(cb2, db2, true, S + d, b_lz, zt_b2, b_air, b_rad, b_forced, b_useF);
            b_cos = cb2.cos_eff;
            b_neg = cb2.alpha;
            add_face(cb2, db2, true, b_air, b_rad, b_forced, S + d, b_useF, hB, qB);
        }
    }

    if constexpr (kChunks) {
        const double T_next_first = from_next_lane(T[0]);
        unsigned int starts = 0;
        if (nm_on && chunky && active) {
#pragma unroll
            for (int j = 0; j < M; j++) {
                const unsigned int vi = (cw[j >> 2] >> (8 * (j & 3))) & (kPalV - 1);
                starts |= (vi >= kPalVMark1 ? vi - (kPalVMark1 - 1) : 0u) << (2 * j);
            }
        }
        while (__any(starts != 0)) {
            if (starts != 0) {
                const int j0 = (__ffs((int)starts) - 1) >> 1;
                const int cn = (int)((starts >> (2 * j0)) & 3u);
                starts &= ~(3u << (2 * j0));
                const int j1 = j0 + cn - 1;
                double ta = T[0], tb = T[0], tp = T_prev_last, tn = T_next_first, up = UL, ui = 0.0, un = 0.0;
#pragma unroll
                for (int j = 0; j < M; j++) {
                    ta = (j == j0) ? +T[j] : +ta;
                    tb = (j == j1) ? +T[j] : +tb;
                    if (j + 1 < M) tp = (j + 1 == j0) ? +T[j] : +tp;
                    if (j > 0) tn = (j == j1 + 1) ? +T[j] : +tn;
                    if (j + 1 < M) up = (j + 1 == j0) ? +U[j] : +up;
                    ui = (j == j0) ? +U[j] : +ui;
                    un = (j == j1) ? +U[j] : +un;
                }
                const bool faceL = is_first && j0 == 0;
                const bool faceR = is_last && j1 == jl;
                const double hL = faceL ? fF_hs : up, hR = faceR ? fB_hs : un;
                const double solA = faceL ? fF_sol : 0.0;
                const double solB = faceR ? fB_sol : 0.0;
                double old_err = 99999.;
                int count = 0;
                for (;;) {
                    const double t_last = (cn == 2) ? tb : ta;
                    const double qL = faceL ? (fF_air * fF_hs + fF_rhs * (fF_rad - ta)) : (up * tp);
                    const double qR = faceR ? (fB_air * fB_hs + fB_rhs * (fB_rad - t_last)) : (un * tn);
                    double x0, x1 = 0.0, err;
                    if (cn == 1) {
                        const double dg = (0.0 + -hL) + -hR;
                        const double q = (((0.0 + qL) + qR) + (solA + solB)) * -1.;
                        x0 = q / dg;
                        err = fabs(x0 - ta);
                    } else {
                        const double u = ui;
                        double dg0 = 0.0 + -u, dg1 = 0.0 - u;
                        const double up0 = 0.0 + u, lo1 = 0.0 + u;
                        dg0 += -hL;
                        dg1 += -hR;
                        const double q0 = ((0.0 + qL) + solA) * -1.;
                        double q1 = ((0.0 + qR) + solB) * -1.;
                        const double f = lo1 / dg0;
                        dg1 -= f * up0;
                        q1 -= f * q0;
                        x1 = q1 / dg1;
                        x0 = (q0 - up0 * x1) / dg0;
                        err = fabs(x0 - ta) + fabs(x1 - tb);
                    }
                    nm_passes++;
                    if (err > old_err) break;
                    if (err != err) { bad |= FLAG_NAN_NOMASS; break; }
                    ta = (ta + x0) * 0.5;
                    if (cn == 2) tb = (tb + x1) * 0.5;
                    const double tol = (count < 100) ? 0.01 : 0.5;
                    if (err / (double)cn < tol) break;
                    old_err = err;
                    count++;
                }
#pragma unroll
                for (int j = 0; j < M; j++) {
                    T[j] = (j == j0) ? ta : T[j];
                    if (j > 0) T[j] = (cn == 2 && j == j1) ? tb : T[j];
                }
            }
        }
    }

    if constexpr (CAV) {
        const double T_next_first = from_next_lane(T[0]);
#pragma unroll
        for (int r = 0; r < 2; r++) {
            const int node = r ? cavref.z : cavref.x;
            const int cidx = r ? cavref.w : cavref.y;
            const int jc = node - seg * M;
            if (active && cidx >= 0 && jc >= 0 && jc < M) {
                double ta = T[0], tb = T_next_first;
#pragma unroll
                for (int j = 0; j < M; j++) {
                    ta = (j == jc) ? +T[j] : +ta;
                    if (j + 1 < M) tb = (j == jc) ? +T[j + 1] : +tb;
                }
                const double u = cavity_u_value(na.cavs[cidx], ta, tb, bad);
#pragma unroll
                for (int j = 0; j < M; j++) U[j] = (j == jc) ? u : U[j];
            }
        }
        UL = from_prev_lane(U[M - 1]);
        if (is_first) UL = 0.0;
    }

    {
        const double hBe = is_last ? hB : 0.0;
        if (full) {
            U[M - 1] = is_last ? hB : U[M - 1];
        } else {
#pragma unroll
            for (int j = 0; j < M; j++) U[j] = (j == jl) ? U[j] + hBe : U[j];
        }
        const double ULe = is_first ? hF : UL;
        const double qFe = is_first ? qF : 0.0;
        const double qBe = is_last ? qB : 0.0;
#ifdef HEAT_STREAM_STAMPS
        asm volatile("" : "+v"(T[0]), "+v"(T[M - 1]));
        HEAT_SSTAMP(6, false);
#endif
        if (full) {
            rk4_horner<M>(T, Vat, U, ULe, is_first, is_last, qFe, [&](int j) -> double { return (j == M - 1) ? qBe : 0.0; });
        } else {
            rk4_horner<M>(T, Vat, U, ULe, is_first, is_last, qFe, [&](int j) -> double { return (j == jl) ? qBe : 0.0; });
        }
#ifdef HEAT_STREAM_STAMPS
        asm volatile("" : "+v"(T[0]), "+v"(T[M - 1]));
        HEAT_SSTAMP(7, false);
#endif
        if constexpr (FUSED) {
            if (full) {
                U[M - 1] = is_last ? 0.0 : U[M - 1];
            } else {
#pragma unroll
                for (int j = 0; j < M; j++) U[j] = (is_last && j == jl) ? 0.0 : U[j];
            }
        }
    }

    if constexpr (!FUSED) {
        if (active) {
            double2 *pT = reinterpret_cast<double2 *>(na.T + tile.node_base);
#pragma unroll
            for (int jp = 0; jp < M / 2; jp++) pT[jp * Lk + lane] = make_double2(T[2 * jp], T[2 * jp + 1]);
        }
    }

    const double T0n = wave_quirk ? shfl_f64(T[0], first_lane) : T[0];
    const double Tln = pick_last(T);
    const double Tnn = Tln;
    {
        const double surf_t = (my_back && !my_useF) ? Tnn : T0n;
        const double hs = conv(my_air, my_forced, c.cos_eff, c.alpha, sidx, surf_t);
        const double face_t = my_back ? Tln : T[0];
        o_hs = hs;
        o_flow = (face_t - my_air) * hs;
        if constexpr (!FUSED) {
            if (active && (is_first || is_last) && (kind_n_mine & 3) == KIND_SPACE) {
                ZoneContrib z;
                z.ha = hs * c.forced;
                z.t_face = face_t;
                sd.zc[__double_as_longlong(s_pos[threadIdx.x])] = z;
            }
        }
        if constexpr (FUSED) {
            if (active && (is_first || is_last) && (c.kind_n & 3) == KIND_SPACE)
                s_hT[fl.slots[(my_back ? kLanes : 0) + wib * kWave + lane]] = make_double2(hs * my_area, face_t);
        }
    }
    if (single) {
        const double hs = conv(b_air, b_forced, b_cos, b_neg, S + d, b_useF ? T0n : Tnn);
        o2_hs = hs;
        o2_flow = (Tln - b_air) * hs;
        if constexpr (!FUSED) {
            if (active) put_zone_contrib(sd, cb2, hs, Tln);
        } else {
            if (active && (cb2.kind_n & 3) == KIND_SPACE)
                s_hT[fl.slots[kLanes + wib * kWave + lane]] = make_double2(hs * my_area, Tln);
        }
    } else if (!(is_first || is_last)) {
        bad = 0;
    }
    bad_all |= bad;

    if constexpr (FUSED) {
        int sidx_next = sidx;
        asm volatile("" : "+v"(sidx_next));
        c_cur = sd.sc[sidx_next];
        dy_cur = sd.dyn[sidx_next];
        if constexpr (SMALL == 2) {
            TeamCtx tcx = team;
            tcx.it = it;
            fused_zone_phase<1>(blk, fa, fl, wib, blk_waves, lane, bad_all, tcx);
        } else {
            fused_zone_phase<0>(blk, fa, fl, wib, blk_waves, lane, bad_all, team);
        }
    }
    }
    HEAT_STAMP(2, false);
    HEAT_SSTAMP(2, false);

    if constexpr (FUSED) {
        if (active) {
            double2 *pT = reinterpret_cast<double2 *>(na.T + tile.node_base);
#pragma unroll
            for (int jp = 0; jp < M / 2; jp++) pT[jp * Lk + lane] = make_double2(T[2 * jp], T[2 * jp + 1]);
        }
        if (threadIdx.x < blk.n_zones) fa.zone_T[fa.zones[blk.first_zone + threadIdx.x]] = s_zT[threadIdx.x];
    }
    if (write_out && active && (is_first || is_last)) {
        SideOut o;
        o.hs = o_hs;
        o.flow = o_flow;
        sd.out[sidx] = o;
    }
    if (write_out && single && active) {
        SideOut o;
        o.hs = o2_hs;
        o.flow = o2_flow;
        sd.out[S + d] = o;
    }
    if (active && bad_all) report_failure(flags, bad_all, (unsigned int)d);
#ifdef HEAT_STAMPS
    asm volatile("s_waitcnt vmcnt(0)" ::: "memory");
#endif
    HEAT_STAMP(3, false);
    HEAT_SSTAMP(3, true);
    HEAT_STAMP(5, true);
    if constexpr (NM) {
        unsigned int tot = nm_passes;
#pragma unroll
        for (int o = kWave / 2; o > 0; o >>= 1) tot += __shfl_down(tot, o, kWave);
        if (lane == 0 && tot) nomass_iters[counter_index] += tot;
    }
}

template <int M, int NM, int PAL, int CAV, int FUSED, int SMALL = 0>
__global__ void __launch_bounds__(FUSED ? 64 * FUSED : 256, (FUSED || (M == 16 && !CAV)) ? 2 : 1)
k_surfaces_fast(const FastTile *__restrict__ tiles, int n_tiles, NodeArrays na, SideArrays sd,
                const StepWeather *__restrict__ weather, const int *__restrict__ step_ptr, int step_fixed,
                const double *__restrict__ zone_T, int *__restrict__ flags,
                unsigned long long *__restrict__ nomass_iters, FusedArgs fa) {
    static_assert(!FUSED || (PAL && !(CAV && M == 16)),
                  "the cluster-resident march exists for palette classes; with gas cavities for 4 or 8 nodes per lane");
    constexpr int kMaxW = FUSED ? FUSED : 4;
    constexpr int kLanes = kMaxW * kWave;
    extern __shared__ double s_dyn[];
    __shared__ double s_pos_static[FUSED ? 2 : kLanes];
    double *const s_pal = s_dyn;
    constexpr bool kVinLds = FUSED && M == 16;
    double *const s_V = s_dyn + kLanes * na.pal_stride;
    FusedLds fl;
    fl.hT = reinterpret_cast<double2 *>(s_V + (kVinLds ? M : 0) * kLanes);
    fl.zT = reinterpret_cast<double *>(fl.hT) + 4 * kLanes;
    fl.za0 = fl.zT + kFusedMaxZones;
    fl.zb0 = fl.za0 + kFusedMaxZones;
    fl.zvol = fl.zb0 + kFusedMaxZones;
    fl.zsa = fl.zvol + kFusedMaxZones;
    fl.zsb = fl.zsa + kFusedMaxZones;
    fl.zoff = reinterpret_cast<int *>(fl.zsb + kFusedMaxZones);
    fl.slots = reinterpret_cast<unsigned short *>(fl.zoff + kFusedMaxZones + 2);
    const int lane = threadIdx.x & (kWave - 1);
    const int wib = threadIdx.x >> 6;
    int wave0 = blockIdx.x * (blockDim.x >> 6) + wib;
    int n_waves = gridDim.x * (blockDim.x >> 6);
    FusedBlock blk{0, 0, 0, 0, 0, 0};
    int blk_waves = 0;
    int bi = blockIdx.x;
    __shared__ int s_next_block;
    const int n_it = FUSED ? fa.n_sub : 1;
    const int step0 = FUSED ? 0 : ((step_fixed >= 0) ? step_fixed : *step_ptr);
    const bool write_out = FUSED || step_fixed >= 0 || step0 == step_ptr[1];
    constexpr bool kTeam = FUSED && SMALL == 2;
    TeamCtx team{0, 0, 0, 0, flags};
    int sb = 0, n_teams = 1;
    if constexpr (kTeam) {
        team.team = (int)blockIdx.x / fa.team_size;
        team.member = (int)blockIdx.x % fa.team_size;
        n_teams = (int)gridDim.x / fa.team_size;
        sb = team.team;
    }
    for (int wave = wave0; FUSED ? (kTeam ? (sb < fa.n_super) : (bi < fa.n_blocks)) : (wave < n_tiles); wave += n_waves) {
    if constexpr (FUSED) {
        if constexpr (kTeam) {
            const FusedSuper su = fa.supers[fa.reverse ? fa.n_super - 1 - sb : sb];
            if (team.member >= su.n_members) {
                sb += n_teams;
                team.round++;
                continue;
            }
            bi = su.first_block + team.member;
        }
        blk = fa.blocks[(!kTeam && fa.reverse) ? fa.n_blocks - 1 - bi : bi];
        blk_waves = blk.n_tiles + (SMALL == 1 ? blk.n_small : 0);
        const bool looping = kTeam || fa.queue != nullptr;
        if (wib >= blk_waves) {
            if (!looping) return;
            for (int q = 0; q < kFusedBarriersAtInit; q++) __syncthreads();
            for (int it = 0; it < fa.n_sub; it++)
                for (int q = 0; q < kFusedBarriersPerSubstep; q++) __syncthreads();
            goto next_block;
        }
        if constexpr (SMALL == 1) {
            if (wib >= blk.n_tiles) {
                fused_small_wave(blk, fa, fl, kLanes, wib, blk_waves, lane, na, sd, weather, flags);
                if (!looping) return;
                goto next_block;
            }
        }
        wave = blk.first_tile + wib;
    }
    {
    const int tix = (!FUSED && fa.reverse) ? n_tiles - 1 - wave : wave;
    const FastTile tl = tiles[tix];
    fast_tile_march<M, NM, PAL, CAV, FUSED, SMALL>(tl, tix, true, lane, wib, s_pal, s_V, s_pos_static, fl, blk, blk_waves, n_it, step0, na,
                                                   sd, site_weather(weather, sd, tl.surf_base), zone_T, flags, nomass_iters, fa,
                                                   write_out, team);
    }
next_block:
    if constexpr (FUSED) {
        if constexpr (kTeam) {
            __syncthreads();
            sb += n_teams;
            team.round++;
        } else {
            if (fa.queue == nullptr) break;
            __syncthreads();
            if (threadIdx.x == 0) s_next_block = (int)(gridDim.x + atomicAdd(fa.queue, 1u));
            __syncthreads();
            bi = s_next_block;
        }
    }
    }
}

constexpr int kTileKindShift = 9;
constexpr int kTileNmBit = 1 << 11;
enum { kStreamWide = 0, kStreamLight = 1, kStreamChunks = 2, kStreamCav = 3 };
template <int VARIANT>
__global__ void __launch_bounds__(256, VARIANT == kStreamLight ? 3 : 2)
k_surfaces_stream(const FastTile *__restrict__ tiles, int n_tiles, NodeArrays na, int64_t gen_base, SideArrays sd,
                  const StepWeather *__restrict__ weather, const int *__restrict__ step_ptr, int step_fixed,
                  const double *__restrict__ zone_T, int *__restrict__ flags,
                  unsigned long long *__restrict__ nomass_iters, int reverse) {
    extern __shared__ double s_pal[];
    __shared__ double s_pos[4 * kWave];
    const int lane = threadIdx.x & (kWave - 1);
    const int wib = threadIdx.x >> 6;
    const int wave0 = blockIdx.x * (blockDim.x >> 6) + wib;
    const int n_waves = gridDim.x * (blockDim.x >> 6);
    const int step0 = (step_fixed >= 0) ? step_fixed : *step_ptr;
    const bool write_out = step_fixed >= 0 || step0 == step_ptr[1];
    const FusedLds fl{};
    const FusedBlock blk{0, 0, 0, 0, 0, 0};
    const FusedArgs fa{};
    if (wave0 >= n_tiles) return;
    constexpr int kNm = VARIANT == kStreamChunks ? 2 : 1;
    const int last = n_tiles - 1;
    FastTile tile_next = tiles[__builtin_amdgcn_readfirstlane(reverse ? last - wave0 : wave0)];
    int site_next = sd.site ? tile_site(sd, tile_next.surf_base) : 0;
    for (int wv = wave0; wv < n_tiles; wv += n_waves) {
        const int w = __builtin_amdgcn_readfirstlane(reverse ? last - wv : wv);
        FastTile tile = tile_next;
        const StepWeather *const wt = weather + (int64_t)site_next * sd.wstride;
        const int wn = min(wv + n_waves, last);
        tile_next = tiles[__builtin_amdgcn_readfirstlane(reverse ? last - wn : wn)];
        const int kind = (tile.k >> kTileKindShift) & 3;
        const bool nm = (tile.k & kTileNmBit) != 0;
        tile.k = (int16_t)(tile.k & (0x1ff | kTileMixedBit | kTileChunkyBit));
        if constexpr (VARIANT == kStreamWide) {
            fast_tile_march<16, 0, 1, 0, 0>(tile, w, false, lane, wib, s_pal, nullptr, s_pos, fl, blk, 0, 1, step0, na, sd, wt,
                                            zone_T, flags, nomass_iters, fa, write_out);
        } else {
            constexpr int kCav = VARIANT == kStreamCav ? 1 : 0;
            switch (kind) {
            case 1:
                fast_tile_march<8, kNm, 1, kCav, 0>(tile, w, nm, lane, wib, s_pal, nullptr, s_pos, fl, blk, 0, 1, step0, na, sd, wt,
                                                    zone_T, flags, nomass_iters, fa, write_out);
                break;
            case 0:
                fast_tile_march<4, kNm, 1, kCav, 0>(tile, w, nm, lane, wib, s_pal, nullptr, s_pos, fl, blk, 0, 1, step0, na, sd, wt,
                                                    zone_T, flags, nomass_iters, fa, write_out);
                break;
            default: {
                unsigned int tot = small_tile_march<kCav>(tile.node_base, tile.surf_base, tile.G, lane, na, gen_base, sd,
                                                          wt[step0],
                                                          zone_T, flags);
#pragma unroll
                for (int o = kWave / 2; o > 0; o >>= 1) tot += __shfl_down(tot, o, kWave);
                if (lane == 0 && tot) nomass_iters[w] += tot;
                break;
            }
            }
        }
        if (sd.site) site_next = tile_site(sd, tile_next.surf_base);
    }
}

#pragma clang fp contract(off)
__global__ void __launch_bounds__(256)
k_surfaces_general(const GeneralTile *__restrict__ tiles, int n_tiles, NodeArrays na, int64_t gen_base,
                   SideArrays sd, const CavityDev *__restrict__ cavs, double *__restrict__ scratch,
                   const StepWeather *__restrict__ weather, const int *__restrict__ step_ptr, int step_fixed,
                   const double *__restrict__ zone_T, int *__restrict__ flags,
                   unsigned long long *__restrict__ nomass_iters) {
    const int lane = threadIdx.x & (kWave - 1);
    const int wave = blockIdx.x * (blockDim.x >> 6) + (threadIdx.x >> 6);
    if (wave >= n_tiles) return;
    const GeneralTile tile = tiles[wave];
    if (lane >= tile.G) return;
    const int d = tile.surf_base + lane;
    const int S = sd.S;

    const SideConst cf = sd.sc[d];
    const SideConst cb = sd.sc[S + d];
    const SideDyn df = sd.dyn[d];
    const SideDyn db = sd.dyn[S + d];
    const int nn = cf.kind_n >> 16;
    const int bk = cb.kind_n & 3;
    const int step = (step_fixed >= 0) ? step_fixed : *step_ptr;
    const StepWeather w = site_weather(weather, sd, tile.surf_base)[step];

    double *Tg = na.T + tile.node_base + lane;
    const double *Vg = na.V + tile.node_base + lane;
    const double *Ug = na.U + tile.node_base + lane;
    const int64_t gofs = tile.node_base - gen_base + lane;
    const double *Fa = na.alpha_f + gofs;
    const double *Ba = na.alpha_b + gofs;
    const double *Mg = na.mass + gofs;
    const int32_t *Cg = na.cav + gofs;
    const int nmax = tile.n_max;
    double *Sx = scratch + tile.scratch_base + lane;
#define SC(a, i) Sx[((int64_t)(a) * nmax + (i)) * kWave]
#define TT(i) Tg[(int64_t)(i) * kWave]
    enum { LO = 0, DG = 1, UP = 2, QQ = 3, AUX = 4, KN = 5, ACC = 6 };

    int bad = 0;
    const double t_front_b = boundary_temperature(cf, w, zone_T);
    const double t_back_b = boundary_temperature(cb, w, zone_T);

    const double T0 = TT(0), Tn = TT(nn - 1);
    const bool quirk = (bk == KIND_AMBIENT);
    double f_hs, f_rad, b_hs, b_rad;
    const double f_surf = T0;
    const double b_surf = quirk ? T0 : Tn;
    eval_side(cf, w, t_front_b, t_front_b, df.rad_t, f_surf, f_hs, f_rad, bad);
    eval_side(cb, w, t_back_b, quirk ? t_front_b : t_back_b, db.rad_t, b_surf, b_hs, b_rad, bad);
    if (f_hs != f_hs || b_hs != b_hs) bad |= FLAG_NAN_HS;
    if (sd.hs_fix != nullptr) {
        const double ff = sd.hs_fix[d], fb = sd.hs_fix[S + d];
        if (ff == ff) f_hs = ff;
        if (fb == fb) b_hs = fb;
    }
    const double f_air = t_front_b, b_air = t_back_b;
    const double f_radhs = rad_hs(cf.emis, f_rad, f_surf);
    const double b_radhs = rad_hs(cb.emis, b_rad, b_surf);

    const double solar_front = df.solar, solar_back = db.solar;
    auto solar = [&](int i) {
        double s = Fa[(int64_t)i * kWave] * solar_front;
        s += Ba[(int64_t)i * kWave] * solar_back;
        return s;
    };
    auto uval = [&](int gidx, double ta, double tb) {
        const int cidx = Cg[(int64_t)gidx * kWave];
        if (cidx >= 0) return cavity_u_value(cavs[cidx], ta, tb, bad);
        return Ug[(int64_t)gidx * kWave];
    };
    auto get_k_q = [&](int ini, int fin) {
        const int nc = fin - ini;
        for (int li = 0; li < nc; li++) { SC(LO, li) = 0.0; SC(DG, li) = 0.0; SC(UP, li) = 0.0; SC(QQ, li) = 0.0; }
        for (int li = 0; li < nc - 1; li++) {
            const int gi = ini + li;
            const double u = uval(gi, TT(gi), TT(gi + 1));
            SC(DG, li) += -u;
            SC(DG, li + 1) = SC(DG, li + 1) - u;
            SC(UP, li) = SC(UP, li) + u;
            SC(LO, li + 1) = SC(LO, li + 1) + u;
        }
        double hf, fq;
        if (ini == 0) {
            const double ts = TT(0);
            fq = f_air * f_hs + f_radhs * (f_rad - ts);
            hf = f_hs;
        } else {
            const double tb = TT(ini - 1), ta = TT(ini);
            const double u = uval(ini - 1, tb, ta);
            hf = u;
            fq = u * tb;
        }
        SC(QQ, 0) += fq;
        SC(DG, 0) += -hf;
        double hb, bq;
        if (fin == nn) {
            const double ts = TT(fin - 1);
            bq = b_air * b_hs + b_radhs * (b_rad - ts);
            hb = b_hs;
        } else {
            const double tb = TT(fin - 1), ta = TT(fin);
            const double u = uval(fin - 1, tb, ta);
            hb = u;
            bq = u * ta;
        }
        SC(QQ, nc - 1) += bq;
        SC(DG, nc - 1) += -hb;
    };
    auto matvec = [&](int li, int nc, auto xfn) {
        double a = 0.0;
        if (li > 0) a += SC(LO, li) * xfn(li - 1);
        a += SC(DG, li) * xfn(li);
        if (li < nc - 1) a += SC(UP, li) * xfn(li + 1);
        return a;
    };

    unsigned long long iters = 0;
    for (int i = 0; i < nn;) {
        if (Mg[(int64_t)i * kWave] >= kMassThreshold) { i++; continue; }
        const int ini = i;
        while (i < nn && Mg[(int64_t)i * kWave] < kMassThreshold) i++;
        const int fin = i, nc = fin - ini;
        double old_err = 99999.;
        int count = 0;
        for (;;) {
            get_k_q(ini, fin);
            iters++;
            for (int li = 0; li < nc; li++) SC(QQ, li) = (SC(QQ, li) + solar(ini + li)) * -1.;
            for (int li = 1; li < nc; li++) {
                const double f = SC(LO, li) / SC(DG, li - 1);
                SC(DG, li) -= f * SC(UP, li - 1);
                SC(QQ, li) -= f * SC(QQ, li - 1);
            }
            SC(QQ, nc - 1) = SC(QQ, nc - 1) / SC(DG, nc - 1);
            for (int li = nc - 2; li >= 0; li--) SC(QQ, li) = (SC(QQ, li) - SC(UP, li) * SC(QQ, li + 1)) / SC(DG, li);
            double err = 0.0;
            for (int li = 0; li < nc; li++) err += fabs(SC(QQ, li) - TT(ini + li));
            if (err > old_err) break;
            if (err != err) { bad |= FLAG_NAN_NOMASS; break; }
            for (int li = 0; li < nc; li++) TT(ini + li) = (TT(ini + li) + SC(QQ, li)) * 0.5;
            const double tol = (count < 100) ? 0.01 : 0.5;
            if (err / (double)nc < tol) break;
            old_err = err;
            count++;
        }
    }

    for (int i = 0; i < nn;) {
        if (Mg[(int64_t)i * kWave] < kMassThreshold) { i++; continue; }
        const int ini = i;
        while (i < nn && Mg[(int64_t)i * kWave] >= kMassThreshold) i++;
        const int fin = i, nc = fin - ini;
        get_k_q(ini, fin);
        for (int li = 0; li < nc; li++) {
            const double v = Vg[(int64_t)(ini + li) * kWave];
            SC(QQ, li) = (SC(QQ, li) + solar(ini + li)) * v;
            if (li > 0) SC(LO, li) *= v;
            SC(DG, li) *= v;
            if (li < nc - 1) SC(UP, li) *= v;
        }
        auto xT = [&](int li) { return TT(ini + li); };
        auto xA = [&](int li) { return SC(AUX, li); };
        for (int li = 0; li < nc; li++) SC(KN, li) = matvec(li, nc, xT) + SC(QQ, li);
        for (int li = 0; li < nc; li++) {
            const double k1 = SC(KN, li), t = TT(ini + li);
            SC(AUX, li) = k1 * 0.5 + t;
            SC(ACC, li) = t + k1 / 6.;
        }
        for (int li = 0; li < nc; li++) SC(KN, li) = matvec(li, nc, xA) + SC(QQ, li);
        for (int li = 0; li < nc; li++) {
            const double k2 = SC(KN, li), t = TT(ini + li);
            SC(AUX, li) = k2 * 0.5 + t;
            SC(ACC, li) += k2 / 3.;
        }
        for (int li = 0; li < nc; li++) SC(KN, li) = matvec(li, nc, xA) + SC(QQ, li);
        for (int li = 0; li < nc; li++) {
            const double k3 = SC(KN, li), t = TT(ini + li);
            SC(AUX, li) = k3 + t;
            SC(ACC, li) += k3 / 3.;
        }
        for (int li = 0; li < nc; li++) SC(KN, li) = matvec(li, nc, xA) + SC(QQ, li);
        for (int li = 0; li < nc; li++) TT(ini + li) = SC(ACC, li) + SC(KN, li) / 6.;
    }

    {
        const double T0n = TT(0), Tnn = TT(nn - 1);
        double fh, bh, r_;
        eval_side(cf, w, t_front_b, t_front_b, df.rad_t, T0n, fh, r_, bad);
        eval_side(cb, w, t_back_b, t_back_b, db.rad_t, quirk ? T0n : Tnn, bh, r_, bad);
        if (fh != fh || bh != bh) bad |= FLAG_NAN_HS;
        if (sd.hs_fix != nullptr) {
            const double ff = sd.hs_fix[d], fb = sd.hs_fix[S + d];
            if (ff == ff) fh = ff;
            if (fb == fb) bh = fb;
        }
        SideOut of, ob;
        of.hs = fh; of.flow = (T0n - t_front_b) * fh;
        ob.hs = bh; ob.flow = (Tnn - t_back_b) * bh;
        sd.out[d] = of;
        sd.out[S + d] = ob;
        put_zone_contrib(sd, cf, fh, T0n);
        put_zone_contrib(sd, cb, bh, Tnn);
    }
    if (bad) report_failure(flags, bad, (unsigned int)d);
    if (iters) nomass_iters[(int64_t)wave * kWave + lane] += iters;
#undef SC
#undef TT
}
#pragma clang fp contract(fast)


template <int ROWS>
__global__ void __launch_bounds__(256)
k_zones(const int64_t *__restrict__ zone_off, const ZoneEntry *__restrict__ entries,
        const ZoneContrib *__restrict__ zc,
        const double *__restrict__ a0, const double *__restrict__ b0, const double *__restrict__ zone_vol,
        double *__restrict__ zone_T, double *__restrict__ partial, int n_zones, double dt,
        int *__restrict__ step_ptr, int *__restrict__ flags, int mode, const int32_t *__restrict__ zlist,
// ... 565 lines not shown
    dyn[rec].rad_t = ir_to_rad_temperature(v);
}

__device__ __forceinline__ double series_value(int b, uint32_t i, const double *__restrict__ T, const SideOut *__restrict__ out,
                                               const double *__restrict__ zone_T) {
    const double *base = b == kProbeBufT ? T : (b == kProbeBufOut ? reinterpret_cast<const double *>(out) : zone_T);
    return base[i];
}

template <int STRIDE>
__device__ __forceinline__ double series_group_lane(const SeriesGroupsDev &g, uint32_t first, uint32_t end, const double *__restrict__ T,
                                                    const SideOut *__restrict__ out, const double *__restrict__ zone_T) {
    double acc = 0.0;
    if (g.weight != nullptr) {
#pragma unroll 4
        for (uint32_t e = first; e < end; e += STRIDE) {
            const double p = g.weight[e] * series_value(g.buf[e], g.idx[e], T, out, zone_T);
            acc = acc + p;
        }
    } else {
#pragma unroll 4
        for (uint32_t e = first; e < end; e += STRIDE) acc = acc + series_value(g.buf[e], g.idx[e], T, out, zone_T);
    }
    return acc;
}

__global__ void __launch_bounds__(256)
k_series_groups(SeriesGroupsDev g, const double *__restrict__ T, const SideOut *__restrict__ out, const double *__restrict__ zone_T) {
    const int lane = threadIdx.x & (kWave - 1);
    const int w = blockIdx.x * (256 / kWave) + (threadIdx.x >> 6);
    if (w < g.n_wave) {
        const uint32_t *seg = g.wave_seg + 3 * (size_t)w;
        const uint32_t e0 = seg[0], e1 = seg[1];
        const double total = wave_sum_f64(series_group_lane<kWave>(g, e0 + lane, e1, T, out, zone_T));
        if (lane == 0) g.part[seg[2]] = total;
        return;
    }
    const int r = (w - g.n_wave) * 4 + (lane >> 4);
    uint32_t e0 = 0, e1 = 0, p = 0;
    if (r < g.n_row) {
        const uint32_t *seg = g.row_seg + 3 * (size_t)r;
        e0 = seg[0], e1 = seg[1], p = seg[2];
    }
    const double total = row_sum_f64(series_group_lane<16>(g, e0 + (lane & 15), e1, T, out, zone_T));
    if ((lane & 15) == 15 && r < g.n_row) g.part[p] = total;
}

__global__ void __launch_bounds__(256)
k_series_stats(SeriesStatsDev s, const double *__restrict__ T, const SideOut *__restrict__ out, const double *__restrict__ zone_T,
               double *__restrict__ group_row, int64_t step) {
    const int64_t q = (int64_t)blockIdx.x * blockDim.x + threadIdx.x;
    if (q >= s.n_probes + s.n_groups) return;
    double v;
    if (q < s.n_probes) {
        v = series_value(s.buf[q], s.idx[q], T, out, zone_T);
    } else {
        const int64_t g = q - s.n_probes;
        const uint32_t p0 = s.part_off[g], p1 = s.part_off[g + 1];
        v = p0 < p1 ? s.part[p0] : 0.0;
        for (uint32_t p = p0 + 1; p < p1; p++) v = v + s.part[p];
        if (group_row != nullptr) group_row[g] = v;
    }
    if (s.q_min != nullptr && v < s.q_min[q]) {
        s.q_min[q] = v;
        if (s.q_step_min != nullptr) s.q_step_min[q] = step;
    }
    if (s.q_max != nullptr && v > s.q_max[q]) {
        s.q_max[q] = v;
        if (s.q_step_max != nullptr) s.q_step_max[q] = step;
    }
    if (s.q_sum != nullptr) s.q_sum[q] = s.q_sum[q] + v;
    if (s.q_lo != nullptr) {
        const double lo = s.q_lo[q];
        if (v < lo) {
            if (s.q_n_below != nullptr) s.q_n_below[q] += 1;
            if (s.q_deg_below != nullptr) s.q_deg_below[q] = s.q_deg_below[q] + (lo - v);
        }
    }
    if (s.q_hi != nullptr) {
        const double hi = s.q_hi[q];
        if (v > hi) {
            if (s.q_n_above != nullptr) s.q_n_above[q] += 1;
            if (s.q_deg_above != nullptr) s.q_deg_above[q] = s.q_deg_above[q] + (v - hi);
        }
    }
}

__global__ void __launch_bounds__(256)
k_series_th_stats(int n, SeriesThStatsDev t, const uint8_t *__restrict__ mode, const double *__restrict__ applied_row) {
    const int i = blockIdx.x * blockDim.x + threadIdx.x;
    if (i >= n) return;
    const int m = mode[i];
    if (t.steps_heating != nullptr && m == 1) t.steps_heating[i] += 1;
    if (t.steps_cooling != nullptr && m == 2) t.steps_cooling[i] += 1;
    if (t.switches != nullptr) {
        if (m != t.prev[i]) t.switches[i] += 1;
        t.prev[i] = (uint8_t)m;
    }
    if (t.sum_heating != nullptr || t.sum_cooling != nullptr) {
        const double a = applied_row[i];
        if (t.sum_heating != nullptr && a > 0.0) t.sum_heating[i] = t.sum_heating[i] + a;
        if (t.sum_cooling != nullptr && a < 0.0) t.sum_cooling[i] = t.sum_cooling[i] + a;
    }
}

__global__ void __launch_bounds__(256)
k_series_air_paths(int n_zones, AirPathsDev ap, const double *__restrict__ row, const double *__restrict__ zone_T,
                   double *__restrict__ a0, double *__restrict__ b0, double *__restrict__ q_row, int *__restrict__ flags) {
#pragma clang fp contract(off)
    const int z = blockIdx.x * blockDim.x + threadIdx.x;
    if (z >= n_zones) return;
    const int p0 = ap.off[z], p1 = ap.off[z + 1];
    if (p0 == p1) return;
    double a = a0[z], b = b0[z];
    const bool clean = a == a && b == b;
    const double tt = zone_T[z];
    for (int i = p0; i < p1; i++) {
        const int orig = ap.orig[i], src = ap.source[i], oc = ap.open_chan[i];
        const double ts = src >= 0 ? zone_T[src] : row[ap.temp_chan[i]];
        bool open = true, switched = false;
        if (oc >= 0) {
            const double set = row[oc], d = ap.half_band[i], s = ap.sense[i];
            const int before = ap.state[orig];
            const double e = s * (tt - set);
            const double g = s * (tt - ts);
            int now = before;
            if (e > d && g > ap.min_delta[i]) now = 1;
            else if (before == 1 && (e < -d || g <= 0.0)) now = 0;
            switched = now != before;
            if (switched) ap.state[orig] = (uint8_t)now;
            open = now == 1;
        }
        double q = 0.0;
        if (open) {
            const double v = ap.volume_gain[i] * row[ap.volume_chan[i]];
            const double tk = ts + 273.15;
            const double rho = 101325. * 28.97 / (8314.46261815324 * tk);
            const double cp = 1002.7370 + 1.2324e-2 * tk;
            const double m = (rho * v) * cp;
            const double mt = m * ts;
            a = a + mt;
            b = b + m;
            const double dt = ts - tt;
            q = m * dt;
        }
        if (q_row != nullptr) q_row[orig] = q;
        if (ap.sum_q != nullptr) ap.sum_q[orig] = ap.sum_q[orig] + q;
        if (ap.steps_open != nullptr && open) ap.steps_open[orig] += 1;
        if (ap.switches != nullptr && switched) ap.switches[orig] += 1;
    }
    a0[z] = a;
    b0[z] = b;
    if (clean && (a != a || b != b)) report_failure(flags, FLAG_NAN_ZONE, (unsigned int)z);
}

__global__ void __launch_bounds__(256) k_fill_f64(double *__restrict__ dst, int64_t n, double value) {
    const int64_t i = (int64_t)blockIdx.x * blockDim.x + threadIdx.x;
    if (i < n) dst[i] = value;
}

__global__ void __launch_bounds__(256) k_series_ideal_begin(IdealLoadsDev il, const double *__restrict__ row) {
    const int i = blockIdx.x * blockDim.x + threadIdx.x;
    if (i >= il.n_loads) return;
    const int hc = il.heat_chan[i], cc = il.cool_chan[i];
    il.setpoint[i] = hc >= 0 ? row[hc] : __builtin_nan("");
    il.setpoint[il.n_loads + i] = cc >= 0 ? row[cc] : __builtin_nan("");
    il.qsum[i] = 0.0;
}

__global__ void __launch_bounds__(256)
k_zone_update_ideal(const double *__restrict__ partial, const double *__restrict__ a0, const double *__restrict__ b0,
                    const double *__restrict__ zone_vol, double *__restrict__ zone_T, int n_zones, double dt,
                    int *__restrict__ step_ptr, int *__restrict__ flags, IdealLoadsDev il) {
    const int z = blockIdx.x * blockDim.x + threadIdx.x;
    if (z == 0) *step_ptr += 1;
    if (z >= n_zones) return;
    const int i = il.load_of_zone[z];
    const double a = partial[z] + a0[z];
    const double b = partial[n_zones + z] + b0[z];
    const double tc = zone_T[z];
    const double cz = zone_mcp(zone_vol[z], tc);
    double q = 0.0, ft = tc;
    if (fabs(b) > 1e-9) {
        const double r = a / b;
        const double nbdt = (-b) * dt;
        const double E = exp(nbdt / cz);
        const double dE = (tc - r) * E;
        const double free_t = r + dE;
        ft = free_t;
        const double D = 1.0 - E;
        if (i >= 0 && D > 0.0) {
            const double h = il.setpoint[i], c = il.setpoint[il.n_loads + i];
            const double tcE = tc * E;
            if (il.heat_chan[i] >= 0 && free_t < h) {
                const double num = b * (h - tcE);
                const double need = num / D - a;
                const double cap = il.heat_cap[i];
                q = need > cap ? cap : need;
                if (!(q > 0.0)) q = 0.0;
                if (q > 0.0) {
                    if (q == need) {
                        ft = h;
                    } else {
                        const double a2 = a + q;
                        const double r2 = a2 / b;
                        const double d2 = (tc - r2) * E;
                        ft = r2 + d2;
                        if (il.n_sat_heating != nullptr) il.n_sat_heating[i] += 1;
                    }
                }
            } else if (il.cool_chan[i] >= 0 && free_t > c) {
                const double num = b * (c - tcE);
                const double need = num / D - a;
                const double cap = -il.cool_cap[i];
                q = need < cap ? cap : need;
                if (!(q < 0.0)) q = 0.0;
                if (q < 0.0) {
                    if (q == need) {
                        ft = c;
                    } else {
                        const double a2 = a + q;
                        const double r2 = a2 / b;
                        const double d2 = (tc - r2) * E;
                        ft = r2 + d2;
                        if (il.n_sat_cooling != nullptr) il.n_sat_cooling[i] += 1;
                    }
                }
            }
        }
    }
    if (ft != ft) report_failure(flags, FLAG_NAN_ZONE, (unsigned int)z);
    zone_T[z] = ft;
    if (i >= 0) il.qsum[i] = il.qsum[i] + q;
}

__global__ void __launch_bounds__(256) k_series_ideal_end(IdealLoadsDev il, double *__restrict__ q_row, int64_t step) {
    const int i = blockIdx.x * blockDim.x + threadIdx.x;
    if (i >= il.n_loads) return;
    const double v = il.qsum[i];
    if (q_row != nullptr) q_row[i] = v;
    if (il.sum_heating != nullptr && v > 0.0) il.sum_heating[i] = il.sum_heating[i] + v;
    if (il.sum_cooling != nullptr && v < 0.0) il.sum_cooling[i] = il.sum_cooling[i] + v;
    if (il.peak_heating != nullptr && v > il.peak_heating[i]) {
        il.peak_heating[i] = v;
        if (il.step_peak_heating != nullptr) il.step_peak_heating[i] = step;
    }
    if (il.peak_cooling != nullptr && v < il.peak_cooling[i]) {
        il.peak_cooling[i] = v;
        if (il.step_peak_cooling != nullptr) il.step_peak_cooling[i] = step;
    }
}
#pragma clang fp contract(fast)

static inline int blocks_for_waves(int n_waves) { return (n_waves + 3) / 4; }
static inline size_t pal_lds_bytes(const NodeArrays &na) { return (size_t)4 * kWave * na.pal_stride * sizeof(double); }

void launch_surfaces_fast(int M, int nm, int pal, int cav, double grid_share, const FastTile *tiles, int n_tiles,
                          const NodeArrays &na,
                          const SideArrays &sa, const StepWeather *weather, const int *step_ptr, int step_fixed,
                          const double *zone_T, int *flags, unsigned long long *nomass_iters, int n_cu, hipStream_t st, int reverse) {
    if (n_tiles <= 0) return;
    static const int tune = getenv("HEAT_AMD_PERSIST") ? atoi(getenv("HEAT_AMD_PERSIST")) : 1;
    const int blocks_per_cu = (M == 4 ? 5 : (M == 8 ? 3 : 2)) * tune;
    const int full_grid = blocks_for_waves(n_tiles);
    const bool persistent = tune > 0 && grid_share > 0.999 && M >= 8;
    const dim3 grid(persistent ? std::min(full_grid, n_cu * blocks_per_cu) : full_grid), block(256);
    FusedArgs no_fa{};
    no_fa.reverse = reverse;
#define HEAT_LAUNCH_FAST(MM, NN, PP, CC)                                                                          \
    hipLaunchKernelGGL((k_surfaces_fast<MM, NN, PP, CC, 0>), grid, block, PP ? pal_lds_bytes(na) : 0, st, tiles, n_tiles, na, sa, weather, \
                       step_ptr, step_fixed, zone_T, flags, nomass_iters, no_fa)
#define HEAT_LAUNCH_M(MM)                                     \
    switch ((nm ? 3 : 0) + (cav ? 2 : (pal ? 1 : 0))) {       \
    case 0: HEAT_LAUNCH_FAST(MM, 0, 0, 0); break;             \
    case 1: HEAT_LAUNCH_FAST(MM, 0, 1, 0); break;             \
    case 2: HEAT_LAUNCH_FAST(MM, 0, 1, 1); break;             \
    case 3: HEAT_LAUNCH_FAST(MM, 1, 0, 0); break;             \
    case 4: if (nm == 2) HEAT_LAUNCH_FAST(MM, 2, 1, 0); else HEAT_LAUNCH_FAST(MM, 1, 1, 0); break; \
    default: if (nm == 2) HEAT_LAUNCH_FAST(MM, 2, 1, 1); else HEAT_LAUNCH_FAST(MM, 1, 1, 1); break; \
    }
    if (M == 4) { HEAT_LAUNCH_M(4) } else if (M == 8) { HEAT_LAUNCH_M(8) } else { HEAT_LAUNCH_M(16) }
#undef HEAT_LAUNCH_M
#undef HEAT_LAUNCH_FAST
}

void launch_surfaces_stream(int variant, const FastTile *tiles, int n_tiles, const NodeArrays &na, int64_t gen_base, const SideArrays &sa,
                            const StepWeather *weather, const int *step_ptr, int step_fixed, const double *zone_T,
                            int *flags, unsigned long long *nomass_iters, int n_cu, hipStream_t st, int reverse) {
    if (n_tiles <= 0) return;
    static const int per_cu_env = getenv("HEAT_AMD_STREAM_BLOCKS") ? atoi(getenv("HEAT_AMD_STREAM_BLOCKS")) : 0;
    const int per_cu = per_cu_env > 0 ? per_cu_env : (variant == kStreamLight ? 3 : 2);
    const int grid = std::min(blocks_for_waves(n_tiles), n_cu * per_cu);
#define HEAT_LAUNCH_STREAM(V)                                                                                       \
    hipLaunchKernelGGL(k_surfaces_stream<V>, dim3(grid), dim3(256), pal_lds_bytes(na), st, tiles, n_tiles, na, gen_base, sa, weather, \
                       step_ptr, step_fixed, zone_T, flags, nomass_iters, reverse)
    if (variant == kStreamWide) HEAT_LAUNCH_STREAM(kStreamWide);
    else if (variant == kStreamLight) HEAT_LAUNCH_STREAM(kStreamLight);
    else if (variant == kStreamChunks) HEAT_LAUNCH_STREAM(kStreamChunks);
    else HEAT_LAUNCH_STREAM(kStreamCav);
#undef HEAT_LAUNCH_STREAM
}

size_t fused_lds_bytes(int max_waves, int M, int pal_stride) {
    return (size_t)max_waves * kWave * ((pal_stride + (M == 16 ? M : 0)) * sizeof(double) + 2 * sizeof(double2)) +
           6 * kFusedMaxZones * sizeof(double) + (kFusedMaxZones + 2) * sizeof(int) + kFusedMaxEntries * sizeof(uint16_t);
}

template <int MM, int NN, int CC, int FW, int SM>
static hipError_t launch_fused_one(int grid_blocks, const FastTile *tiles, int n_tiles, const NodeArrays &na,
                                   const SideArrays &sa, const StepWeather *weather, int *flags,
                                   unsigned long long *nomass_iters, const FusedArgs &fa, hipStream_t st) {
    const size_t lds = fused_lds_bytes(FW, MM, na.pal_stride);
    constexpr int kMaxDevices = 64;
    static std::atomic<size_t> attr_bytes[kMaxDevices];
    if (lds > 160 * 1024) return hipErrorInvalidValue;
    int dev = 0;
    if (hipGetDevice(&dev) != hipSuccess || dev < 0 || dev >= kMaxDevices) dev = kMaxDevices - 1;
    if (lds > 64 * 1024 && lds > attr_bytes[dev].load(std::memory_order_acquire)) {
        hipError_t e = hipFuncSetAttribute(reinterpret_cast<const void *>(&k_surfaces_fast<MM, NN, 1, CC, FW, SM>),
                                           hipFuncAttributeMaxDynamicSharedMemorySize, (int)lds);
        if (e != hipSuccess) return e;
        if (dev != kMaxDevices - 1) attr_bytes[dev].store(lds, std::memory_order_release);
    }
    hipLaunchKernelGGL((k_surfaces_fast<MM, NN, 1, CC, FW, SM>), dim3(grid_blocks), dim3(kWave * FW), lds, st, tiles,
                       n_tiles, na, sa, weather, nullptr, 0, nullptr, flags, nomass_iters, fa);
    return hipSuccess;
}

int fused_blocks_per_cu(int M, int cav, int mixed, int max_waves, int pal_stride) {
    const int waves_per_simd = (M == 4 && !cav && !mixed) ? 3 : 2;
    const int by_regs = std::max(1, waves_per_simd * 4 / max_waves);
    const int by_lds = std::max<int>(1, (int)(160 * 1024 / fused_lds_bytes(max_waves, M, pal_stride)));
    return std::min(by_regs, by_lds);
}

template <int MM, int NN>
static int team_occupancy(size_t lds) {
    int n = 0;
    if (hipOccupancyMaxActiveBlocksPerMultiprocessor(&n, reinterpret_cast<const void *>(&k_surfaces_fast<MM, NN, 1, 0, 4, 2>),
                                                     kWave * 4, lds) != hipSuccess)
        return 0;
    return n;
}
int fused_team_blocks_per_cu(int M, int nm, int pal_stride) {
    const size_t lds = fused_lds_bytes(4, M, pal_stride);
    if (M == 4) return nm ? team_occupancy<4, 1>(lds) : team_occupancy<4, 0>(lds);
    if (M == 8) return nm ? team_occupancy<8, 1>(lds) : team_occupancy<8, 0>(lds);
    return nm ? team_occupancy<16, 1>(lds) : team_occupancy<16, 0>(lds);
}

hipError_t launch_surfaces_fused(int M, int nm, int cav, int mixed, int max_waves, int grid_blocks, const FastTile *tiles,
                                 int n_tiles, const NodeArrays &na, const SideArrays &sa, const StepWeather *weather,
                                 int *flags, unsigned long long *nomass_iters, const FusedArgs &fa, hipStream_t st) {
    const int n_blocks = grid_blocks;
    if (n_blocks <= 0) return hipSuccess;
    if (cav && M == 16) return hipErrorInvalidValue;
#define HEAT_FUSED(MM, NN, CC, FW, SM) \
    launch_fused_one<MM, NN, CC, FW, SM>(n_blocks, tiles, n_tiles, na, sa, weather, flags, nomass_iters, fa, st)
    if (mixed == 2) {
        if (cav || max_waves > 4) return hipErrorInvalidValue;
        if (M == 4) return nm ? HEAT_FUSED(4, 1, 0, 4, 2) : HEAT_FUSED(4, 0, 0, 4, 2);
        if (M == 8) return nm ? HEAT_FUSED(8, 1, 0, 4, 2) : HEAT_FUSED(8, 0, 0, 4, 2);
        return nm ? HEAT_FUSED(16, 1, 0, 4, 2) : HEAT_FUSED(16, 0, 0, 4, 2);
    }
    if (mixed) {
        if (M == 4) return max_waves <= 4 ? HEAT_FUSED(4, 1, 1, 4, 1) : HEAT_FUSED(4, 1, 1, 8, 1);
        if (M == 8) return max_waves <= 4 ? HEAT_FUSED(8, 1, 1, 4, 1) : HEAT_FUSED(8, 1, 1, 8, 1);
        return max_waves <= 4 ? HEAT_FUSED(16, 1, 0, 4, 1) : HEAT_FUSED(16, 1, 0, 8, 1);
    }
    if (nm == 2 && !cav && M <= 8) {
        if (M == 4) return max_waves <= 4 ? HEAT_FUSED(4, 2, 0, 4, 0) : HEAT_FUSED(4, 2, 0, 8, 0);
        return max_waves <= 4 ? HEAT_FUSED(8, 2, 0, 4, 0) : HEAT_FUSED(8, 2, 0, 8, 0);
    }
#define HEAT_FUSED_NW(MM, CC)                                                    \
    (max_waves <= 4 ? (nm ? HEAT_FUSED(MM, 1, CC, 4, 0) : HEAT_FUSED(MM, 0, CC, 4, 0)) \
                    : (nm ? HEAT_FUSED(MM, 1, CC, 8, 0) : HEAT_FUSED(MM, 0, CC, 8, 0)))
    if (M == 4) return cav ? HEAT_FUSED_NW(4, 1) : HEAT_FUSED_NW(4, 0);
    if (M == 8) return cav ? HEAT_FUSED_NW(8, 1) : HEAT_FUSED_NW(8, 0);
    return HEAT_FUSED_NW(16, 0);
#undef HEAT_FUSED_NW
#undef HEAT_FUSED
}

void launch_surfaces_general(const GeneralTile *tiles, int n_tiles, const NodeArrays &na, int64_t gen_base,
                             const SideArrays &sa, const CavityDev *cavs, double *scratch,
                             const StepWeather *weather, const int *step_ptr, int step_fixed,
                             const double *zone_T, int *flags, unsigned long long *nomass_iters, hipStream_t st) {
    if (n_tiles <= 0) return;
    hipLaunchKernelGGL(k_surfaces_general, dim3(blocks_for_waves(n_tiles)), dim3(256), 0, st, tiles, n_tiles, na,
                       gen_base, sa, cavs, scratch, weather, step_ptr, step_fixed, zone_T, flags, nomass_iters);
}

void launch_surfaces_small(int with_cavities, const GeneralTile *tiles, int n_tiles, const NodeArrays &na,
                           int64_t gen_base, const SideArrays &sa, const CavityDev *cavs,
                           const StepWeather *weather, const int *step_ptr, int step_fixed, const double *zone_T,
                           int *flags, unsigned long long *nomass_iters, hipStream_t st) {
    if (n_tiles <= 0) return;
    if (with_cavities)
        hipLaunchKernelGGL(k_surfaces_small<1>, dim3(blocks_for_waves(n_tiles)), dim3(256), 0, st, tiles, n_tiles, na,
                           gen_base, sa, cavs, weather, step_ptr, step_fixed, zone_T, flags, nomass_iters);
    else
        hipLaunchKernelGGL(k_surfaces_small<0>, dim3(blocks_for_waves(n_tiles)), dim3(256), 0, st, tiles, n_tiles, na,
                           gen_base, sa, cavs, weather, step_ptr, step_fixed, zone_T, flags, nomass_iters);
}

void launch_zones(const int64_t *zone_off, const ZoneEntry *entries, const ZoneContrib *zc,
                  const double *a0, const double *b0, const double *zone_vol, double *zone_T, double *partial,
                  int n_zones, double dt, int *step_ptr, int *flags, int mode, const int32_t *zlist, int n_list,
                  const int32_t *slot_of, int n_shared, int rows, hipStream_t st) {
    const int n_z = (mode == 2 || mode == 3) ? n_list : n_zones;
    if (mode == 2 && n_z <= 0) return;
    if (rows) {
        const int nb = n_z > 0 ? (n_z + 15) / 16 : 1;
        hipLaunchKernelGGL(k_zones<1>, dim3(nb), dim3(256), 0, st, zone_off, entries, zc, a0, b0, zone_vol, zone_T,
                           partial, n_zones, dt, step_ptr, flags, mode, zlist, n_list, slot_of, n_shared);
    } else {
        const int nb = n_z > 0 ? blocks_for_waves(n_z) : 1;
        hipLaunchKernelGGL(k_zones<0>, dim3(nb), dim3(256), 0, st, zone_off, entries, zc, a0, b0, zone_vol, zone_T,
                           partial, n_zones, dt, step_ptr, flags, mode, zlist, n_list, slot_of, n_shared);
    }
}

void launch_zone_update_shared(const double *gathered, int n_blocks, const int32_t *shared_zone, int n_shared,
                               const double *a0, const double *b0, const double *zone_vol, double *zone_T,
                               double dt, int *flags, hipStream_t st) {
    if (n_shared <= 0) return;
    hipLaunchKernelGGL(k_zone_update_shared, dim3((n_shared + 255) / 256), dim3(256), 0, st, gathered, n_blocks,
                       shared_zone, n_shared, a0, b0, zone_vol, zone_T, dt, flags);
}

void launch_zone_update(const double *gathered, int n_blocks, const double *a0, const double *b0,
                        const double *zone_vol, double *zone_T, int n_zones, double dt, int *step_ptr,
                        int *flags, hipStream_t st) {
    const int nb = n_zones > 0 ? (n_zones + 255) / 256 : 1;
    hipLaunchKernelGGL(k_zone_update, dim3(nb), dim3(256), 0, st, gathered, n_blocks, a0, b0, zone_vol, zone_T,
                       n_zones, dt, step_ptr, flags);
}

void launch_nodes_fast(int M, const FastTile *tiles, int n_tiles, double *Tbuf, const int32_t *meta,
                       const int64_t *first_slot, double *state, int to_state, const uint8_t *cls, hipStream_t st) {
    if (n_tiles <= 0) return;
    const dim3 grid(blocks_for_waves(n_tiles)), block(256);
    switch (M) {
    case 4: hipLaunchKernelGGL(k_nodes_fast<4>, grid, block, 0, st, tiles, n_tiles, Tbuf, meta, first_slot, state, to_state, cls); break;
    case 8: hipLaunchKernelGGL(k_nodes_fast<8>, grid, block, 0, st, tiles, n_tiles, Tbuf, meta, first_slot, state, to_state, cls); break;
    default: hipLaunchKernelGGL(k_nodes_fast<16>, grid, block, 0, st, tiles, n_tiles, Tbuf, meta, first_slot, state, to_state, cls); break;
    }
}

void launch_nodes_general(const GeneralTile *tiles, int n_tiles, double *Tbuf, const int32_t *meta,
                          const int64_t *first_slot, double *state, int to_state, hipStream_t st) {
    if (n_tiles <= 0) return;
    hipLaunchKernelGGL(k_nodes_general, dim3(blocks_for_waves(n_tiles)), dim3(256), 0, st, tiles, n_tiles, Tbuf,
                       meta, first_slot, state, to_state);
}

void launch_surf_scalars(int n_surf, const SlotArrays &sl, SideDyn *dyn, SideOut *out, const double *side_alpha,
                         double *state, int to_state, int what, hipStream_t st) {
    if (n_surf <= 0) return;
    hipLaunchKernelGGL(k_surf_scalars, dim3((n_surf + 255) / 256), dim3(256), 0, st, n_surf, sl, dyn, out, side_alpha,
                       state, to_state, what);
}

void launch_zone_scalars(int n_zones, const int64_t *zone_slot, double *zone_T, double *state, int to_state,
                         hipStream_t st) {
    if (n_zones <= 0) return;
    hipLaunchKernelGGL(k_zone_scalars, dim3((n_zones + 255) / 256), dim3(256), 0, st, n_zones, zone_slot, zone_T,
                       state, to_state);
}

void launch_inputs_compact(int n_surf, int n_zones, const double *in, const double *side_alpha, SideDyn *dyn, double *zone_T,
                           const SlotArrays &sl, double *mirror, hipStream_t st) {
    const int n = std::max(n_surf, n_zones);
    if (n <= 0) return;
    hipLaunchKernelGGL(k_inputs_compact, dim3((n + 255) / 256), dim3(256), 0, st, n_surf, n_zones, in, side_alpha, dyn, zone_T,
                       sl, mirror);
}

void launch_outputs_compact(int n_surf, int n_zones, const SideOut *out, const int32_t *orig_of, const double *zone_T,
                            double *dst, hipStream_t st) {
    const int n = std::max(n_surf, n_zones);
    if (n <= 0) return;
    hipLaunchKernelGGL(k_outputs_compact, dim3((n + 255) / 256), dim3(256), 0, st, n_surf, n_zones, out, orig_of, zone_T, dst);
}

void launch_begin_march(const StepWeather *h_weather, StepWeather *weather, int n_sub, int n_records, const double *h_zone_ab,
                        double *a0, double *b0, int n_zones, int *step_ptr, hipStream_t st) {
    const int n = std::max(std::max(n_records, n_zones), 1);
    hipLaunchKernelGGL(k_begin_march, dim3((n + 255) / 256), dim3(256), 0, st, h_weather, weather, n_records, h_zone_ab, a0, b0,
                       n_zones, step_ptr, n_sub - 1);
}

void launch_series_inputs(int n_surf, const double *row, const SeriesInputs &in, const double *T, const double *side_alpha,
                          SideDyn *dyn, const SlotArrays &sl, double *mirror, hipStream_t st) {
    if (n_surf <= 0) return;
    hipLaunchKernelGGL(k_series_inputs, dim3((n_surf + 255) / 256), dim3(256), 0, st, n_surf, row, in, T, side_alpha, dyn, sl, mirror);
}

void launch_series_sky(int n_surf, const SkyRecord *records, const SeriesSky &sky, const double *side_alpha, SideDyn *dyn,
                       const SlotArrays &sl, double *mirror, hipStream_t st) {
    if (n_surf <= 0) return;
    hipLaunchKernelGGL(k_series_sky, dim3((n_surf + 255) / 256), dim3(256), 0, st, n_surf, records, sky, side_alpha, dyn, sl, mirror);
}

void launch_series_shading(const SkyRecord *records, const SeriesShades &sh, double *sunlit_row, hipStream_t st) {
    if (sh.n <= 0) return;
    hipLaunchKernelGGL(k_series_shading, dim3((sh.n + 255) / 256), dim3(256), 0, st, records, sh, sunlit_row);
}

void launch_series_apertures(const SkyRecord *records, const SeriesApertures &ap, double *transmitted, hipStream_t st) {
    if (ap.n <= 0) return;
    hipLaunchKernelGGL(k_series_apertures, dim3((ap.n + 255) / 256), dim3(256), 0, st, records, ap, transmitted);
}

void launch_series_solar_gains(int n_surf, const SeriesGains &g, const double *side_alpha, SideDyn *dyn, const SlotArrays &sl,
                               double *mirror, hipStream_t st) {
    if (g.n_receivers <= 0) return;
    hipLaunchKernelGGL(k_series_solar_gains, dim3((g.n_receivers + 255) / 256), dim3(256), 0, st, n_surf, g, side_alpha, dyn, sl, mirror);
}

void launch_series_emission(const SeriesRoomRadiation &rr, const double *T, hipStream_t st) {
    if (rr.n_emitters <= 0) return;
    hipLaunchKernelGGL(k_series_emission, dim3((rr.n_emitters + 255) / 256), dim3(256), 0, st, rr, T);
}

void launch_series_room_radiation(int n_surf, const SeriesRoomRadiation &rr, const double *row, SideDyn *dyn, const SlotArrays &sl,
                                  double *mirror, double *irradiance_row, hipStream_t st) {
    if (rr.n_receivers <= 0) return;
    hipLaunchKernelGGL(k_series_room_radiation, dim3((rr.n_receivers + 255) / 256), dim3(256), 0, st, n_surf, rr, row, dyn, sl, mirror,
                       irradiance_row);
}

void launch_series_zone_loads(int n_zones, const ZoneLoadsDev &zl, const double *row, const double *zone_T, double *a0, double *b0,
                              double *applied_row, int *flags, hipStream_t st) {
    if (n_zones <= 0) return;
    hipLaunchKernelGGL(k_series_zone_loads, dim3((n_zones + 255) / 256), dim3(256), 0, st, n_zones, zl, row, zone_T, a0, b0, applied_row,
                       flags);
}

void launch_series_probe(int64_t n_probes, const uint8_t *buf, const uint32_t *idx, const double *T, const SideOut *out,
                         const double *zone_T, double *trace_row, const int *flags, int *fail_step, int step, hipStream_t st) {
    const int64_t n = std::max<int64_t>(n_probes, 1);
    hipLaunchKernelGGL(k_series_probe, dim3((unsigned int)((n + 255) / 256)), dim3(256), 0, st, n_probes, buf, idx, T, out, zone_T,
                       trace_row, flags, fail_step, step);
}

void launch_series_groups(const SeriesGroupsDev &g, const double *T, const SideOut *out, const double *zone_T, hipStream_t st) {
    const int n_waves = g.n_wave + (g.n_row + 3) / 4;
    if (n_waves <= 0) return;
    hipLaunchKernelGGL(k_series_groups, dim3(blocks_for_waves(n_waves)), dim3(256), 0, st, g, T, out, zone_T);
}

void launch_series_stats(const SeriesStatsDev &s, const double *T, const SideOut *out, const double *zone_T, double *group_row,
                         int64_t step, hipStream_t st) {
    const int64_t n = s.n_probes + s.n_groups;
    if (n <= 0) return;
    hipLaunchKernelGGL(k_series_stats, dim3((unsigned int)((n + 255) / 256)), dim3(256), 0, st, s, T, out, zone_T, group_row, step);
}

void launch_series_th_stats(int n_thermostats, const SeriesThStatsDev &t, const uint8_t *mode, const double *applied_row, hipStream_t st) {
    if (n_thermostats <= 0) return;
    hipLaunchKernelGGL(k_series_th_stats, dim3((n_thermostats + 255) / 256), dim3(256), 0, st, n_thermostats, t, mode, applied_row);
}

void launch_series_air_paths(int n_zones, const AirPathsDev &ap, const double *row, const double *zone_T, double *a0, double *b0,
                             double *q_row, int *flags, hipStream_t st) {
    if (n_zones <= 0) return;
    hipLaunchKernelGGL(k_series_air_paths, dim3((n_zones + 255) / 256), dim3(256), 0, st, n_zones, ap, row, zone_T, a0, b0, q_row, flags);
}

void launch_fill_f64(double *dst, int64_t n, double value, hipStream_t st) {
    if (n <= 0) return;
    hipLaunchKernelGGL(k_fill_f64, dim3((unsigned int)((n + 255) / 256)), dim3(256), 0, st, dst, n, value);
}

void launch_series_ideal_begin(const IdealLoadsDev &il, const double *row, hipStream_t st) {
    if (il.n_loads <= 0) return;
    hipLaunchKernelGGL(k_series_ideal_begin, dim3((il.n_loads + 255) / 256), dim3(256), 0, st, il, row);
}

void launch_zone_update_ideal(const double *partial, const double *a0, const double *b0, const double *zone_vol, double *zone_T,
                              int n_zones, double dt, int *step_ptr, int *flags, const IdealLoadsDev &il, hipStream_t st) {
    const int nb = n_zones > 0 ? (n_zones + 255) / 256 : 1;
    hipLaunchKernelGGL(k_zone_update_ideal, dim3(nb), dim3(256), 0, st, partial, a0, b0, zone_vol, zone_T, n_zones, dt, step_ptr,
                       flags, il);
}

void launch_series_ideal_end(const IdealLoadsDev &il, double *q_row, int64_t step, hipStream_t st) {
    if (il.n_loads <= 0) return;
    hipLaunchKernelGGL(k_series_ideal_end, dim3((il.n_loads + 255) / 256), dim3(256), 0, st, il, q_row, step);
}

void launch_set_step(int *step_ptr, int v, int last, hipStream_t st) {
    hipLaunchKernelGGL(k_set_step, dim3(1), dim3(1), 0, st, step_ptr, v, last);
}

}

#if defined(HEAT_STAMPS) || defined(HEAT_STREAM_STAMPS)
extern "C" int heat_debug_stamps(unsigned long long *dst, int n_blocks) {
    return (int)hipMemcpyFromSymbol(dst, HIP_SYMBOL(heat::g_stamps), (size_t)n_blocks * heat::kStampsPerBlock * sizeof(unsigned long long));
}
#endif
```

heat_amd/csrc/kernels.hpp:

```cpp
#pragma once
#include <hip/hip_runtime.h>
#include "layout.hpp"

namespace heat {

struct SlotArrays {
    const int64_t *hs_f, *hs_b, *flow_f, *flow_b, *solar_f, *solar_b, *ir_f, *ir_b;
};

void launch_surfaces_fast(int M, int nm, int pal, int cav, double grid_share, const FastTile *tiles, int n_tiles,
                          const NodeArrays &na,
                          const SideArrays &sa, const StepWeather *weather, const int *step_ptr, int step_fixed,
                          const double *zone_T, int *flags, unsigned long long *nomass_iters, int n_cu, hipStream_t st, int reverse = 0);
constexpr int kStreamKindShift = 9;
constexpr int kStreamKindSmall = 3;
constexpr int kStreamNmBit = 1 << 11;
constexpr int kStreamVariants = 4;
void launch_surfaces_stream(int variant, const FastTile *tiles, int n_tiles, const NodeArrays &na, int64_t gen_base, const SideArrays &sa,
                            const StepWeather *weather, const int *step_ptr, int step_fixed, const double *zone_T,
                            int *flags, unsigned long long *nomass_iters, int n_cu, hipStream_t st, int reverse = 0);
int fused_blocks_per_cu(int M, int cav, int mixed, int max_waves, int pal_stride);
int fused_team_blocks_per_cu(int M, int nm, int pal_stride);
hipError_t launch_surfaces_fused(int M, int nm, int cav, int mixed, int max_waves, int grid_blocks, const FastTile *tiles, int n_tiles,
                                 const NodeArrays &na, const SideArrays &sa, const StepWeather *weather, int *flags,
                                 unsigned long long *nomass_iters, const FusedArgs &fa, hipStream_t st);
void launch_surfaces_general(const GeneralTile *tiles, int n_tiles, const NodeArrays &na, int64_t gen_base,
                             const SideArrays &sa, const CavityDev *cavs, double *scratch,
                             const StepWeather *weather, const int *step_ptr, int step_fixed,
                             const double *zone_T, int *flags, unsigned long long *nomass_iters, hipStream_t st);
void launch_surfaces_small(int with_cavities, const GeneralTile *tiles, int n_tiles, const NodeArrays &na,
                           int64_t gen_base, const SideArrays &sa, const CavityDev *cavs,
                           const StepWeather *weather, const int *step_ptr, int step_fixed, const double *zone_T,
                           int *flags, unsigned long long *nomass_iters, hipStream_t st);
void launch_zones(const int64_t *zone_off, const ZoneEntry *entries, const ZoneContrib *zc,
                  const double *a0, const double *b0, const double *zone_vol, double *zone_T, double *partial,
                  int n_zones, double dt, int *step_ptr, int *flags, int mode, const int32_t *zlist, int n_list,
                  const int32_t *slot_of, int n_shared, int rows, hipStream_t st);
void launch_zone_update_shared(const double *gathered, int n_blocks, const int32_t *shared_zone, int n_shared,
                               const double *a0, const double *b0, const double *zone_vol, double *zone_T,
                               double dt, int *flags, hipStream_t st);
void launch_zone_update(const double *gathered, int n_blocks, const double *a0, const double *b0,
                        const double *zone_vol, double *zone_T, int n_zones, double dt, int *step_ptr,
                        int *flags, hipStream_t st);
void launch_nodes_fast(int M, const FastTile *tiles, int n_tiles, double *Tbuf, const int32_t *meta,
                       const int64_t *first_slot, double *state, int to_state, const uint8_t *cls, hipStream_t st);
void launch_nodes_general(const GeneralTile *tiles, int n_tiles, double *Tbuf, const int32_t *meta,
                          const int64_t *first_slot, double *state, int to_state, hipStream_t st);
void launch_surf_scalars(int n_surf, const SlotArrays &sl, SideDyn *dyn, SideOut *out, const double *side_alpha,
                         double *state, int to_state, int what, hipStream_t st);
void launch_zone_scalars(int n_zones, const int64_t *zone_slot, double *zone_T, double *state, int to_state,
                         hipStream_t st);
void launch_inputs_compact(int n_surf, int n_zones, const double *in, const double *side_alpha, SideDyn *dyn, double *zone_T,
                           const SlotArrays &sl, double *mirror, hipStream_t st);
void launch_outputs_compact(int n_surf, int n_zones, const SideOut *out, const int32_t *orig_of, const double *zone_T,
                            double *dst, hipStream_t st);
void launch_begin_march(const StepWeather *h_weather, StepWeather *weather, int n_sub, int n_records, const double *h_zone_ab,
                        double *a0, double *b0, int n_zones, int *step_ptr, hipStream_t st);
void launch_set_step(int *step_ptr, int v, int last, hipStream_t st);

struct SeriesInputs {
    const int32_t *chan;
    const double *gain[4];
    const uint8_t *own_face;
    const uint32_t *face;
};
void launch_series_inputs(int n_surf, const double *row, const SeriesInputs &in, const double *T, const double *side_alpha,
                          SideDyn *dyn, const SlotArrays &sl, double *mirror, hipStream_t st);
struct alignas(16) SkyRecord {
    double sun_x, sun_y, sun_z, beam, diffuse, ground, ir_sky, ir_ground;
};
struct ShadeFactors {
    const double *f;
    const double *diffuse;
    const double *ground;
};
struct SeriesSky {
    const uint8_t *mode;
    const double *normal;
    const int32_t *site;
    const double *gain[4];
    const int32_t *shade;
    ShadeFactors sf;
};
struct SeriesShades {
    int n;
    const int32_t *site;
    const int32_t *horizon;
    const double *tab;
    const double *tan2;
    double *f;
};
void launch_series_shading(const SkyRecord *records, const SeriesShades &sh, double *sunlit_row, hipStream_t st);
void launch_series_sky(int n_surf, const SkyRecord *records, const SeriesSky &sky, const double *side_alpha, SideDyn *dyn,
                       const SlotArrays &sl, double *mirror, hipStream_t st);
struct SeriesApertures {
    int n;
    const int32_t *dev;
    const int32_t *site;
    const double *normal;
    const double *coef;
    const double *tau_scale;
    double2 *power;
    double *sum;
    const int32_t *shade;
    ShadeFactors sf;
};
struct SeriesGains {
    int n_receivers;
    const uint32_t *rec;
    const int64_t *slice_off;
    const int32_t *ap;
    const double2 *share;
    const double2 *power;
    const double *gain[2];
};
void launch_series_apertures(const SkyRecord *records, const SeriesApertures &ap, double *transmitted, hipStream_t st);
void launch_series_solar_gains(int n_surf, const SeriesGains &g, const double *side_alpha, SideDyn *dyn, const SlotArrays &sl,
                               double *mirror, hipStream_t st);
struct SeriesRoomRadiation {
    int n_emitters, n_receivers;
    const uint32_t *face;
    double *emission;
    const uint32_t *rec;
    const int32_t *off;
    const int32_t *src;
    const double *factor;
    const double *gain[2];
    double *sum;
};
void launch_series_emission(const SeriesRoomRadiation &rr, const double *T, hipStream_t st);
void launch_series_room_radiation(int n_surf, const SeriesRoomRadiation &rr, const double *row, SideDyn *dyn, const SlotArrays &sl,
                                  double *mirror, double *irradiance_row, hipStream_t st);
struct ZoneLoadsDev {
    const int32_t *off;
    const int32_t *gain_chan;
    const double *gain_factor;
    const int32_t *flow_volume_chan, *flow_temp_chan;
    const double *flow_volume_gain;
    const int32_t *th_sensor, *th_heat_chan, *th_cool_chan, *th_orig;
    const double *th_heat_power, *th_cool_power, *th_half_band;
    uint8_t *th_mode;
};
void launch_series_zone_loads(int n_zones, const ZoneLoadsDev &zl, const double *row, const double *zone_T, double *a0, double *b0,
                              double *applied_row, int *flags, hipStream_t st);
constexpr int kProbeBufT = 0, kProbeBufOut = 1, kProbeBufZone = 2;
void launch_series_probe(int64_t n_probes, const uint8_t *buf, const uint32_t *idx, const double *T, const SideOut *out,
                         const double *zone_T, double *trace_row, const int *flags, int *fail_step, int step, hipStream_t st);

struct SeriesGroupsDev {
    const uint8_t *buf;
    const uint32_t *idx;
    const double *weight;
    const uint32_t *wave_seg;
    const uint32_t *row_seg;
    int n_wave, n_row;
    double *part;
};
void launch_series_groups(const SeriesGroupsDev &g, const double *T, const SideOut *out, const double *zone_T, hipStream_t st);
struct SeriesStatsDev {
    int64_t n_probes, n_groups;
    const uint8_t *buf;
    const uint32_t *idx;
    const double *part;
    const uint32_t *part_off;
    double *q_min, *q_max, *q_sum, *q_deg_below, *q_deg_above;
    int64_t *q_step_min, *q_step_max, *q_n_below, *q_n_above;
    const double *q_lo, *q_hi;
};
void launch_series_stats(const SeriesStatsDev &s, const double *T, const SideOut *out, const double *zone_T, double *group_row,
                         int64_t step, hipStream_t st);
struct SeriesThStatsDev {
    int64_t *steps_heating, *steps_cooling, *switches;
    double *sum_heating, *sum_cooling;
    uint8_t *prev;
};
void launch_series_th_stats(int n_thermostats, const SeriesThStatsDev &t, const uint8_t *mode, const double *applied_row, hipStream_t st);
struct AirPathsDev {
    const int32_t *off;
    const int32_t *source, *temp_chan, *volume_chan, *open_chan, *orig;
    const double *volume_gain, *sense, *half_band, *min_delta;
    uint8_t *state;
    double *sum_q;
    int64_t *steps_open, *switches;
};
void launch_series_air_paths(int n_zones, const AirPathsDev &ap, const double *row, const double *zone_T, double *a0, double *b0,
                             double *q_row, int *flags, hipStream_t st);
void launch_fill_f64(double *dst, int64_t n, double value, hipStream_t st);

struct IdealLoadsDev {
    int n_loads;
    const int32_t *load_of_zone;
    const int32_t *heat_chan, *cool_chan;
    const double *heat_cap, *cool_cap;
    double *setpoint;
    double *qsum;
    int64_t *n_sat_heating, *n_sat_cooling;
    double *sum_heating, *sum_cooling, *peak_heating, *peak_cooling;
    int64_t *step_peak_heating, *step_peak_cooling;
};
void launch_series_ideal_begin(const IdealLoadsDev &il, const double *row, hipStream_t st);
void launch_zone_update_ideal(const double *partial, const double *a0, const double *b0, const double *zone_vol, double *zone_T,
                              int n_zones, double dt, int *step_ptr, int *flags, const IdealLoadsDev &il, hipStream_t st);
void launch_series_ideal_end(const IdealLoadsDev &il, double *q_row, int64_t step, hipStream_t st);

}
```

Measured before the change: 495.8 billion.

## Add lean register-light variant of fused M=16 kernel for three waves per SIMD

```diff
diff --git a/heat_amd/csrc/batch.hip b/heat_amd/csrc/batch.hip
--- a/heat_amd/csrc/batch.hip
+++ b/heat_amd/csrc/batch.hip
@@ -818,7 +818,8 @@
             if (beside_exchange) {
                 const int fw = (g2 & 1) ? 8 : 4;
                 static const int room_env = getenv("HEAT_AMD_FUSED_ROOM") ? atoi(getenv("HEAT_AMD_FUSED_ROOM")) : 0;
-                const int room = room_env > 0 ? room_env : n_cu * fused_blocks_per_cu(kFastM[c], kFastCAV[c], g2 >> 1, fw, b->na.pal_stride);
+                const int nm_v = kFastNM[c] ? ((b->class_has_chunks[c] && !(g2 >> 1) && !kFastCAV[c] && kFastM[c] <= 8) ? 2 : 1) : 0;
+                const int room = room_env > 0 ? room_env : n_cu * fused_blocks_per_cu(kFastM[c], nm_v, kFastCAV[c], g2 >> 1, fw, b->na.pal_stride);
                 const int reserve = reserve_env >= 0 ? reserve_env
                                                      : std::min(room / 2, std::max(fw == 4 ? 16 : 8, (int)(room * streamed_share)));
                 if (nb > room - reserve) {
diff --git a/heat_amd/csrc/device_math.hpp b/heat_amd/csrc/device_math.hpp
--- a/heat_amd/csrc/device_math.hpp
+++ b/heat_amd/csrc/device_math.hpp
@@ -39,6 +39,18 @@
     return (h < 0.1) ? 0.1 : h;
 }
 
+struct NaturalOut {
+    double h;
+    int bad;
+};
+__device__ __attribute__((noinline)) NaturalOut tarp_natural_coef_called(double air_t, double surf_t, double nat_pos, double nat_neg) {
+    NaturalOut o;
+    o.bad = 0;
+    o.h = tarp_natural_coef(air_t, surf_t, nat_pos, nat_neg, o.bad);
+    return o;
+}
+__device__ __attribute__((noinline)) double exp_called(double x) { return exp(x); }
+
 __device__ __forceinline__ double tarp_forced(double air_speed, double area, double perimeter, bool windward) {
     const double wf = windward ? 1.0 : 0.5;
     return 2.537 * wf * 1.67 * sqrt(perimeter * air_speed / area);
@@ -55,8 +67,8 @@
 __device__ __forceinline__ double clamp_solar_front(double s) { return (s != s || s < 0.0) ? 0.0 : s; }
 __device__ __forceinline__ double clamp_solar_back(double s) { return (s != s) ? 0.0 : s; }
 
-__device__ __forceinline__ double rad_hs(double emis, double rad_t, double surf_t) {
-    const double tm = 273.15 + (rad_t + surf_t) / 2.;
+__device__ __forceinline__ double rad_hs(double emis, double rad_t, double surf_t, double kelvin0 = 273.15) {
+    const double tm = kelvin0 + (rad_t + surf_t) / 2.;
     return 4. * emis * kSigma * ((tm * tm) * tm);
 }
 
@@ -79,6 +91,8 @@
 __device__ __forceinline__ double zone_mcp(double volume, double temp) {
     return volume * air_density(temp + 273.15) * air_heat_capacity(temp + 273.15) / 1.;
 }
+
+__device__ __attribute__((noinline)) double zone_mcp_called(double volume, double temp) { return zone_mcp(volume, temp); }
 
 __device__ __forceinline__ double powr(double x, double y) { return exp(y * log(x)); }
 
diff --git a/heat_amd/csrc/kernels.hip b/heat_amd/csrc/kernels.hip
--- a/heat_amd/csrc/kernels.hip
+++ b/heat_amd/csrc/kernels.hip
@@ -115,13 +115,34 @@
     }
 }
 
+template <int STRIDE>
+struct VFromLds {
+    const double *base;
+    int at;
+    __device__ __forceinline__ double operator()(int j) const { return base[at + j * STRIDE]; }
+};
+template <typename VF>
+__device__ __forceinline__ void v_fresh(VF &) {}
+template <unsigned long long BITS>
+__device__ __forceinline__ double local_f64() {
+    int lo, hi;
+    asm volatile("v_mov_b32 %0, %2\n\tv_mov_b32 %1, %3" : "=v"(lo), "=v"(hi) : "i"((int)(BITS & 0xffffffffull)), "i"((int)(BITS >> 32)));
+    return __hiloint2double(hi, lo);
+}
+template <int STRIDE>
+__device__ __forceinline__ void v_fresh(VFromLds<STRIDE> &V) { asm volatile("" : "+v"(V.at)); }
+
 template <int M, typename VF, typename QF>
 __device__ __forceinline__ void rk4_horner(double (&T)[M], VF V, const double (&Ue)[M], double ULe, bool is_first,
                                            bool is_last, double qF, QF qsel) {
     double v[M], z[M];
+    v_fresh(V);
     apply_A<M, true>(T, V, Ue, ULe, is_first, is_last, qF, qsel, [&](int j, double y) { v[j] = y * (1.0 / 24.0); });
+    v_fresh(V);
     apply_A<M, false>(v, V, Ue, ULe, is_first, is_last, qF, qsel, [&](int j, double y) { z[j] = 4.0 * v[j] + y; });
+    v_fresh(V);
     apply_A<M, false>(z, V, Ue, ULe, is_first, is_last, qF, qsel, [&](int j, double y) { z[j] = 12.0 * v[j] + y; });
+    v_fresh(V);
     apply_A<M, false>(z, V, Ue, ULe, is_first, is_last, qF, qsel,
                       [&](int j, double y) { T[j] = (T[j] + 24.0 * v[j]) + y; });
 }
@@ -353,6 +374,12 @@
 }
 #pragma clang fp contract(fast)
 
+__host__ __device__ constexpr bool fused_is_lean(int M, int NM, int CAV, int FUSED, int SMALL) {
+    return FUSED == 4 && M == 16 && !NM && !CAV && SMALL == 0;
+}
+__host__ __device__ constexpr int fused_wave_doubles(int M, int pal_stride) {
+    return kWave * ((M == 16 && pal_stride < M) ? M : pal_stride);
+}
 struct FusedLds {
     double2 *hT;
     double *zT, *za0, *zb0, *zvol;
@@ -383,17 +410,17 @@
     int e_first, n_e, zoff, z, slot0;
     double zT, za0, zb0, zvol;
 };
-__device__ __forceinline__ void fused_pre_a(const FusedBlock &blk, const FusedArgs &fa, FusedPre &p) {
+__device__ __forceinline__ void fused_pre_a(const FusedBlock &blk, const FusedArgs &fa, FusedPre &p, unsigned int tidx) {
     p = FusedPre{0, 0, 0, 0, 0, 0.0, 0.0, 0.0, 0.0};
     const int nz = blk.n_zones;
     if (nz > 0) {
         p.e_first = fa.zone_eoff[blk.first_zone];
         p.n_e = fa.zone_eoff[blk.first_zone + nz];
-        p.zoff = fa.zone_eoff[blk.first_zone + min((int)threadIdx.x, nz)];
-        p.z = fa.zones[blk.first_zone + min((int)threadIdx.x, nz - 1)];
-    }
-}
-__device__ __forceinline__ void fused_pre_b(const FusedBlock &blk, const FusedArgs &fa, FusedPre &p) {
+        p.zoff = fa.zone_eoff[blk.first_zone + min((int)tidx, nz)];
+        p.z = fa.zones[blk.first_zone + min((int)tidx, nz - 1)];
+    }
+}
+__device__ __forceinline__ void fused_pre_b(const FusedBlock &blk, const FusedArgs &fa, FusedPre &p, unsigned int tidx) {
     if (blk.n_zones > 0) {
         p.n_e -= p.e_first;
         p.zoff -= p.e_first;
@@ -401,20 +428,20 @@
         p.za0 = fa.a0[p.z];
         p.zb0 = fa.b0[p.z];
         p.zvol = fa.vol[p.z];
-        if (p.n_e > 0) p.slot0 = fa.slots[p.e_first + min((int)threadIdx.x, p.n_e - 1)];
+        if (p.n_e > 0) p.slot0 = fa.slots[p.e_first + min((int)tidx, p.n_e - 1)];
     }
 }
 __device__ __forceinline__ void fused_block_init(const FusedBlock &blk, const FusedArgs &fa, const FusedLds &l, int n_threads,
-                                                 const FusedPre &p) {
-    if ((int)threadIdx.x <= blk.n_zones) l.zoff[threadIdx.x] = p.zoff;
-    if ((int)threadIdx.x < blk.n_zones) {
-        l.zT[threadIdx.x] = p.zT;
-        l.za0[threadIdx.x] = p.za0;
-        l.zb0[threadIdx.x] = p.zb0;
-        l.zvol[threadIdx.x] = p.zvol;
-    }
-    if ((int)threadIdx.x < p.n_e) l.slots[p.slot0] = (unsigned short)threadIdx.x;
-    for (int e = threadIdx.x + n_threads; e < p.n_e; e += n_threads) l.slots[fa.slots[p.e_first + e]] = (unsigned short)e;
+                                                 const FusedPre &p, unsigned int tidx) {
+    if ((int)tidx <= blk.n_zones) l.zoff[tidx] = p.zoff;
+    if ((int)tidx < blk.n_zones) {
+        l.zT[tidx] = p.zT;
+        l.za0[tidx] = p.za0;
+        l.zb0[tidx] = p.zb0;
+        l.zvol[tidx] = p.zvol;
+    }
+    if ((int)tidx < p.n_e) l.slots[p.slot0] = (unsigned short)tidx;
+    for (int e = tidx + n_threads; e < p.n_e; e += n_threads) l.slots[fa.slots[p.e_first + e]] = (unsigned short)e;
     __syncthreads();
 }
 
@@ -425,7 +452,7 @@
 __device__ __forceinline__ unsigned long long team_granule(unsigned int data, unsigned int tag) {
     return ((unsigned long long)tag << 32) | data;
 }
-template <int TEAM>
+template <int TEAM, int LEAN = 0>
 __device__ __forceinline__ void fused_zone_phase(const FusedBlock &blk, const FusedArgs &fa, const FusedLds &l, int wib,
                                                  int n_waves, int lane, int &bad_all, const TeamCtx &tc_) {
     __syncthreads();
@@ -479,7 +506,7 @@
         a += l.za0[j];
         b += l.zb0[j];
         double ft = tc;
-        if (fabs(b) > 1e-9) ft = a / b + (tc - a / b) * exp(-b * fa.dt / cz);
+        if (fabs(b) > 1e-9) ft = a / b + (tc - a / b) * (LEAN ? exp_called(-b * fa.dt / cz) : exp(-b * fa.dt / cz));
         if (ft != ft) bad_all |= FLAG_NAN_ZONE;
         l.zT[j] = ft;
     };
@@ -488,7 +515,7 @@
             const int j = wib;
             const int e0 = l.zoff[j], e1 = l.zoff[j + 1];
             const double tc = l.zT[j];
-            const double cz = zone_mcp(l.zvol[j], tc);
+            const double cz = LEAN ? zone_mcp_called(l.zvol[j], tc) : zone_mcp(l.zvol[j], tc);
             double a = 0.0, b = 0.0;
             for (int e = e0 + lane; e < e1; e += kWave) {
                 const double2 ht = l.hT[e];
@@ -516,7 +543,7 @@
             const int jj = on ? j : 0;
             const int e0 = l.zoff[jj], e1 = on ? l.zoff[jj + 1] : e0;
             const double tc = l.zT[jj];
-            const double cz = zone_mcp(l.zvol[jj], tc);
+            const double cz = LEAN ? zone_mcp_called(l.zvol[jj], tc) : zone_mcp(l.zvol[jj], tc);
             double a = 0.0, b = 0.0;
             for (int e = e0 + rl; __any(e < e1); e += 16) {
                 if (e < e1) {
@@ -652,7 +679,7 @@
 #endif
 
 template <int M, int NM, int PAL, int CAV, int FUSED, int SMALL = 0>
-__device__ __forceinline__ void fast_tile_march(const FastTile tile, int counter_index, bool nm_on, int lane, int wib,
+__device__ __forceinline__ void fast_tile_march(const FastTile tile, int counter_index, bool nm_on, int lane_in, int wib_in,
                                                 double *s_pal, double *s_V, double *s_pos, const FusedLds &fl, const FusedBlock &blk,
                                                 int blk_waves, int n_it, int step0, const NodeArrays &na,
                                                 const SideArrays &sd, const StepWeather *__restrict__ weather,
@@ -661,15 +688,23 @@
                                                 bool write_out = true, const TeamCtx team = TeamCtx{0, 0, 0, 0, nullptr}) {
     constexpr int kLanes = (FUSED ? FUSED : 4) * kWave;
     constexpr bool kVinLds = FUSED && M == 16;
+    constexpr bool kLean = fused_is_lean(M, NM, CAV, FUSED, SMALL);
+    unsigned int tid0 = threadIdx.x;
+    if constexpr (kLean) asm volatile("" : "+v"(tid0));
+    const int lane = kLean ? (int)(tid0 & (kWave - 1)) : lane_in;
+    const int wib = kLean ? (int)(tid0 >> 6) : wib_in;
+    const unsigned int tidx = kLean ? tid0 : threadIdx.x;
     HEAT_STAMP(4, true);
     HEAT_STAMP(0, false);
     HEAT_SSTAMP(0, false);
     double2 *const s_hT = fl.hT;
     double *const s_zT = fl.zT;
     (void)s_hT; (void)s_zT; (void)s_V; (void)s_pos; (void)nm_on; (void)blk; (void)blk_waves; (void)counter_index;
+    const int v_at = kVinLds ? wib * fused_wave_doubles(M, na.pal_stride) + lane : 0;
+    (void)v_at;
     FusedPre pre;
     (void)pre;
-    if constexpr (FUSED) fused_pre_a(blk, fa, pre);
+    if constexpr (FUSED) fused_pre_a(blk, fa, pre, tidx);
     const bool mixed = PAL && (tile.k & kTileMixedBit) != 0;
     constexpr bool kChunks = NM == 2 && PAL;
     const bool chunky = kChunks && (tile.k & kTileChunkyBit) != 0;
@@ -716,12 +751,12 @@
     double my_area = 0.0;
     if constexpr (FUSED) {
         my_lz = fa.side_lzone[sidx];
-        my_area = fa.side_area[sidx];
+        if constexpr (!kLean) my_area = fa.side_area[sidx];
         if constexpr (kSingleLane) b_lz = single ? fa.side_lzone[S + d] : 0;
     }
     (void)b_lz;
     int peer_lz = 0;
-    if constexpr (FUSED) peer_lz = fa.side_lzone[d];
+    if constexpr (FUSED && !kLean) peer_lz = fa.side_lzone[d];
     (void)peer_lz;
 
     double T[M], V[M], U[M];
@@ -730,7 +765,7 @@
     if constexpr (PAL) {
         const int pstride = na.pal_stride;
         const int ubase = na.pal_ubase;
-        double *sp = s_pal + wib * (kWave * pstride);
+        double *sp = s_pal + wib * (FUSED ? fused_wave_doubles(M, pstride) : kWave * pstride);
         auto load_cls_T = [&]() {
             const unsigned char *pc = na.cls + tile.node_base + (int64_t)ll * M;
             if constexpr (M == 4) {
@@ -752,7 +787,7 @@
         };
         if constexpr (FUSED) {
             load_cls_T();
-            fused_pre_b(blk, fa, pre);
+            fused_pre_b(blk, fa, pre, tidx);
         }
         {
             const double2 *gp = reinterpret_cast<const double2 *>(na.pal + (int64_t)tile.surf_base * pstride);
@@ -786,7 +821,7 @@
         }
         if constexpr (kVinLds) {
 #pragma unroll
-            for (int j = 0; j < M; j++) s_V[j * kLanes + threadIdx.x] = V[j];
+            for (int j = 0; j < M; j++) s_V[v_at + j * kWave] = V[j];
         }
     } else {
         const double2 *pT = reinterpret_cast<const double2 *>(na.T + tile.node_base);
@@ -803,7 +838,7 @@
         }
     }
     HEAT_STAMP(7, false);
-    if constexpr (FUSED) fused_block_init(blk, fa, fl, blk_waves * kWave, pre);
+    if constexpr (FUSED) fused_block_init(blk, fa, fl, blk_waves * kWave, pre, tidx);
 
     const int first_lane = lane - seg;
     const int nn = kind_n_mine >> 16;
@@ -828,7 +863,7 @@
     }
 
     auto Vat = [&](int j) -> double {
-        if constexpr (kVinLds) return s_V[j * kLanes + threadIdx.x];
+        if constexpr (kVinLds) return s_V[v_at + j * kWave];
         else return V[j];
     };
     auto V_last = [&]() {
@@ -855,6 +890,8 @@
     if constexpr (FUSED) w_next = weather[min(it + 1, n_it - 1)];
     const SideConst c = c_cur;
     const SideDyn dy = dy_cur;
+    int rec_it = sidx;
+    if constexpr (kLean) asm volatile("" : "+v"(rec_it));
     auto btemp = [&](const SideConst &cc, int lz, double zt) -> double {
         const int kind = cc.kind_n & 3;
         if (kind == KIND_SPACE) {
@@ -880,7 +917,10 @@
         } else if (back && kind == KIND_AMBIENT) {
             const int fkind = (cc.kind_n >> 4) & 3;
             if (fkind == KIND_SPACE) {
-                if constexpr (FUSED) rad_t = s_zT[peer_lz];
+                if constexpr (kLean) {
+                    rad_t = s_zT[fa.side_lzone[rec - S]];
+                }
+                else if constexpr (FUSED) rad_t = s_zT[peer_lz];
                 else rad_t = zt;
             } else if (fkind == KIND_AMBIENT) {
                 rad_t = cc.forced;
@@ -892,7 +932,14 @@
         (void)rec;
     };
     auto conv = [&](double air_t, double forced, double nat_pos, double nat_neg, int rec, double surf_t) {
-        double hs = forced + tarp_natural_coef(air_t, surf_t, nat_pos, nat_neg, bad);
+        double hs;
+        if constexpr (kLean) {
+            const NaturalOut nat = tarp_natural_coef_called(air_t, surf_t, nat_pos, nat_neg);
+            bad |= nat.bad;
+            hs = forced + nat.h;
+        } else {
+            hs = forced + tarp_natural_coef(air_t, surf_t, nat_pos, nat_neg, bad);
+        }
         if (hs != hs) bad |= FLAG_NAN_HS;
         if (sd.hs_fix != nullptr) {
             const double fix = sd.hs_fix[rec];
@@ -901,7 +948,16 @@
         return hs;
     };
 
-    const double T0 = wave_quirk ? shfl_f64(T[0], first_lane) : T[0];
+    auto from_first = [&](double x) -> double {
+        if constexpr (kLean) {
+            const int lo = __builtin_amdgcn_ds_bpermute(first_lane << 2, __double2loint(x));
+            const int hi = __builtin_amdgcn_ds_bpermute(first_lane << 2, __double2hiint(x));
+            return __hiloint2double(hi, lo);
+        } else {
+            return shfl_f64(x, first_lane);
+        }
+    };
+    const double T0 = wave_quirk ? from_first(T[0]) : T[0];
     const double Tn = pick_last(T);
 
     double UL = from_prev_lane(U[M - 1]);
@@ -920,7 +976,9 @@
         q_out = 0.0;
         const double surf_t = (back && !use_front_T) ? Tn : T0;
         const double hs = conv(air_t, forced, cc.cos_eff, cc.alpha, rec, surf_t);
-        const double rhs = rad_hs(cc.emis, rad_t, surf_t);
+        double kelvin0 = 273.15;
+        if constexpr (kLean) kelvin0 = local_f64<__builtin_bit_cast(unsigned long long, 273.15)>();
+        const double rhs = rad_hs(cc.emis, rad_t, surf_t, kelvin0);
         const double sol = dd.solar;
         if constexpr (NM) {
             if constexpr (kChunks) {
@@ -981,10 +1039,10 @@
 
     double my_air, my_rad, my_forced;
     bool my_useF;
-    prepare(c, dy, my_back, sidx, my_lz, zt_mine, my_air, my_rad, my_forced, my_useF);
+    prepare(c, dy, my_back, rec_it, my_lz, zt_mine, my_air, my_rad, my_forced, my_useF);
     if (is_first || is_last) {
         double h_, q_;
-        add_face(c, dy, my_back, my_air, my_rad, my_forced, sidx, my_useF, h_, q_);
+        add_face(c, dy, my_back, my_air, my_rad, my_forced, rec_it, my_useF, h_, q_);
         hF = my_back ? 0.0 : h_;
         qF = my_back ? 0.0 : q_;
         hB = my_back ? h_ : 0.0;
@@ -1118,7 +1176,14 @@
         asm volatile("" : "+v"(T[0]), "+v"(T[M - 1]));
         HEAT_SSTAMP(6, false);
 #endif
-        if (full) {
+        if constexpr (kLean) {
+            const VFromLds<kWave> Vl{s_V, v_at};
+            if (full) {
+                rk4_horner<M>(T, Vl, U, ULe, is_first, is_last, qFe, [&](int j) -> double { return (j == M - 1) ? qBe : 0.0; });
+            } else {
+                rk4_horner<M>(T, Vl, U, ULe, is_first, is_last, qFe, [&](int j) -> double { return (j == jl) ? qBe : 0.0; });
+            }
+        } else if (full) {
             rk4_horner<M>(T, Vat, U, ULe, is_first, is_last, qFe, [&](int j) -> double { return (j == M - 1) ? qBe : 0.0; });
         } else {
             rk4_horner<M>(T, Vat, U, ULe, is_first, is_last, qFe, [&](int j) -> double { return (j == jl) ? qBe : 0.0; });
@@ -1145,9 +1210,36 @@
         }
     }
 
-    const double T0n = wave_quirk ? shfl_f64(T[0], first_lane) : T[0];
+    const double T0n = wave_quirk ? from_first(T[0]) : T[0];
     const double Tln = pick_last(T);
     const double Tnn = Tln;
+    if constexpr (kLean) {
+        int sidx_next = sidx;
+        asm volatile("" : "+v"(sidx_next));
+        c_cur = sd.sc[sidx_next];
+        const double area = fa.side_area[sidx_next];
+        double air, rad_, forced;
+        bool useF;
+        prepare(c_cur, dy, my_back, sidx_next, my_lz, 0.0, air, rad_, forced, useF);
+        const double surf_t = (my_back && !useF) ? Tnn : T0n;
+        const double hs = conv(air, forced, c_cur.cos_eff, c_cur.alpha, sidx_next, surf_t);
+        const double face_t = my_back ? Tln : T[0];
+        int tid = threadIdx.x;
+        asm volatile("" : "+v"(tid));
+        if (active && (is_first || is_last) && (c_cur.kind_n & 3) == KIND_SPACE)
+            s_hT[fl.slots[(my_back ? kLanes : 0) + tid]] = make_double2(hs * area, face_t);
+        if (it == n_it - 1 && write_out && active && (is_first || is_last)) {
+            SideOut o;
+            o.hs = hs;
+            o.flow = (face_t - air) * hs;
+            sd.out[sidx_next] = o;
+        }
+        if (!(is_first || is_last)) bad = 0;
+        bad_all |= bad;
+        dy_cur = sd.dyn[sidx_next];
+        fused_zone_phase<0, 1>(blk, fa, fl, tid >> 6, blk_waves, tid & (kWave - 1), bad_all, team);
+        continue;
+    }
     {
         const double surf_t = (my_back && !my_useF) ? Tnn : T0n;
         const double hs = conv(my_air, my_forced, c.cos_eff, c.alpha, sidx, surf_t);
@@ -1201,13 +1293,21 @@
 
     if constexpr (FUSED) {
         if (active) {
+            int l_out = lane;
+            if constexpr (kLean) {
+                int tid = threadIdx.x;
+                asm volatile("" : "+v"(tid));
+                l_out = tid & (kWave - 1);
+            }
             double2 *pT = reinterpret_cast<double2 *>(na.T + tile.node_base);
 #pragma unroll
-            for (int jp = 0; jp < M / 2; jp++) pT[jp * Lk + lane] = make_double2(T[2 * jp], T[2 * jp + 1]);
-        }
-        if (threadIdx.x < blk.n_zones) fa.zone_T[fa.zones[blk.first_zone + threadIdx.x]] = s_zT[threadIdx.x];
-    }
-    if (write_out && active && (is_first || is_last)) {
+            for (int jp = 0; jp < M / 2; jp++) pT[jp * Lk + l_out] = make_double2(T[2 * jp], T[2 * jp + 1]);
+        }
+        int t_out = threadIdx.x;
+        if constexpr (kLean) asm volatile("" : "+v"(t_out));
+        if (t_out < blk.n_zones) fa.zone_T[fa.zones[blk.first_zone + t_out]] = s_zT[t_out];
+    }
+    if (!kLean && write_out && active && (is_first || is_last)) {
         SideOut o;
         o.hs = o_hs;
         o.flow = o_flow;
@@ -1219,7 +1319,7 @@
         o.flow = o2_flow;
         sd.out[S + d] = o;
     }
-    if (active && bad_all) report_failure(flags, bad_all, (unsigned int)d);
+    if (active && bad_all) report_failure(flags, bad_all, (unsigned int)(kLean ? sidx - (my_back ? S : 0) : d));
 #ifdef HEAT_STAMPS
     asm volatile("s_waitcnt vmcnt(0)" ::: "memory");
 #endif
@@ -1235,7 +1335,7 @@
 }
 
 template <int M, int NM, int PAL, int CAV, int FUSED, int SMALL = 0>
-__global__ void __launch_bounds__(FUSED ? 64 * FUSED : 256, (FUSED || (M == 16 && !CAV)) ? 2 : 1)
+__global__ void __launch_bounds__(FUSED ? 64 * FUSED : 256, fused_is_lean(M, NM, CAV, FUSED, SMALL) ? 3 : ((FUSED || (M == 16 && !CAV)) ? 2 : 1))
 k_surfaces_fast(const FastTile *__restrict__ tiles, int n_tiles, NodeArrays na, SideArrays sd,
                 const StepWeather *__restrict__ weather, const int *__restrict__ step_ptr, int step_fixed,
                 const double *__restrict__ zone_T, int *__restrict__ flags,
@@ -1247,10 +1347,9 @@
     extern __shared__ double s_dyn[];
     __shared__ double s_pos_static[FUSED ? 2 : kLanes];
     double *const s_pal = s_dyn;
-    constexpr bool kVinLds = FUSED && M == 16;
-    double *const s_V = s_dyn + kLanes * na.pal_stride;
+    double *const s_V = s_dyn;
     FusedLds fl;
-    fl.hT = reinterpret_cast<double2 *>(s_V + (kVinLds ? M : 0) * kLanes);
+    fl.hT = reinterpret_cast<double2 *>(s_dyn + kMaxW * (FUSED ? fused_wave_doubles(M, na.pal_stride) : kWave * na.pal_stride));
     fl.zT = reinterpret_cast<double *>(fl.hT) + 4 * kLanes;
     fl.za0 = fl.zT + kFusedMaxZones;
     fl.zb0 = fl.za0 + kFusedMaxZones;
@@ -1271,6 +1370,9 @@
     const int step0 = FUSED ? 0 : ((step_fixed >= 0) ? step_fixed : *step_ptr);
     const bool write_out = FUSED || step_fixed >= 0 || step0 == step_ptr[1];
     constexpr bool kTeam = FUSED && SMALL == 2;
+    constexpr bool kLeanK = fused_is_lean(M, NM, CAV, FUSED, SMALL);
+    int tile_ix = 0;
+    (void)tile_ix;
     TeamCtx team{0, 0, 0, 0, flags};
     int sb = 0, n_teams = 1;
     if constexpr (kTeam) {
@@ -1307,10 +1409,11 @@
                 goto next_block;
             }
         }
-        wave = blk.first_tile + wib;
+        if constexpr (kLeanK) tile_ix = blk.first_tile + __builtin_amdgcn_readfirstlane(wib);
+        else wave = blk.first_tile + wib;
     }
     {
-    const int tix = (!FUSED && fa.reverse) ? n_tiles - 1 - wave : wave;
+    const int tix = kLeanK ? tile_ix : ((!FUSED && fa.reverse) ? n_tiles - 1 - wave : wave);
     const FastTile tl = tiles[tix];
     fast_tile_march<M, NM, PAL, CAV, FUSED, SMALL>(tl, tix, true, lane, wib, s_pal, s_V, s_pos_static, fl, blk, blk_waves, n_it, step0, na,
                                                    sd, site_weather(weather, sd, tl.surf_base), zone_T, flags, nomass_iters, fa,
@@ -2482,7 +2585,7 @@
 }
 
 size_t fused_lds_bytes(int max_waves, int M, int pal_stride) {
-    return (size_t)max_waves * kWave * ((pal_stride + (M == 16 ? M : 0)) * sizeof(double) + 2 * sizeof(double2)) +
+    return (size_t)max_waves * (fused_wave_doubles(M, pal_stride) * sizeof(double) + kWave * 2 * sizeof(double2)) +
            6 * kFusedMaxZones * sizeof(double) + (kFusedMaxZones + 2) * sizeof(int) + kFusedMaxEntries * sizeof(uint16_t);
 }
 
@@ -2507,8 +2610,8 @@
     return hipSuccess;
 }
 
-int fused_blocks_per_cu(int M, int cav, int mixed, int max_waves, int pal_stride) {
-    const int waves_per_simd = (M == 4 && !cav && !mixed) ? 3 : 2;
+int fused_blocks_per_cu(int M, int nm, int cav, int mixed, int max_waves, int pal_stride) {
+    const int waves_per_simd = ((M == 4 && !cav && !mixed) || fused_is_lean(M, nm, cav, max_waves <= 4 ? 4 : 8, mixed)) ? 3 : 2;
     const int by_regs = std::max(1, waves_per_simd * 4 / max_waves);
     const int by_lds = std::max<int>(1, (int)(160 * 1024 / fused_lds_bytes(max_waves, M, pal_stride)));
     return std::min(by_regs, by_lds);
diff --git a/heat_amd/csrc/kernels.hpp b/heat_amd/csrc/kernels.hpp
--- a/heat_amd/csrc/kernels.hpp
+++ b/heat_amd/csrc/kernels.hpp
@@ -19,7 +19,7 @@
 void launch_surfaces_stream(int variant, const FastTile *tiles, int n_tiles, const NodeArrays &na, int64_t gen_base, const SideArrays &sa,
                             const StepWeather *weather, const int *step_ptr, int step_fixed, const double *zone_T,
                             int *flags, unsigned long long *nomass_iters, int n_cu, hipStream_t st, int reverse = 0);
-int fused_blocks_per_cu(int M, int cav, int mixed, int max_waves, int pal_stride);
+int fused_blocks_per_cu(int M, int nm, int cav, int mixed, int max_waves, int pal_stride);
 int fused_team_blocks_per_cu(int M, int nm, int pal_stride);
 hipError_t launch_surfaces_fused(int M, int nm, int cav, int mixed, int max_waves, int grid_blocks, const FastTile *tiles, int n_tiles,
                                  const NodeArrays &na, const SideArrays &sa, const StepWeather *weather, int *flags,
```

Measured after the change: 488.4 billion. 1.5% lower.
